# THUDM/GCC

Measured on NVIDIA H100. Metric: subgraphs/sec (MoCo pretrain step), higher is better.
Workload: dtype f32

## Files before the change

gcc_b200/csrc/gin_bwd.cu:

```cuda
#include "gin_common.cuh"
#include "tc_gemm.cuh"
#ifndef GCCB_EMU
#include <cuda_bf16.h>
#endif

namespace gccb {

template <int H>
__global__ void __launch_bounds__(256)
gin_pool_predict_bwd_kernel(GinDims d, const int32_t* __restrict__ node_off_v, int B,
                            const float* __restrict__ params, gccb_gin_layout_t lay,
                            const float* __restrict__ score, const float* __restrict__ dfeat,
                            uint64_t drop_key, uint64_t drop_step, int drop_layer_base,
                            uint32_t keep_thresh, int DW, float* __restrict__ dS,
                            float* __restrict__ dpool) {
  constexpr int G = GCCB_GPB;
  __shared__ float ds[G][H];
  __shared__ float dsl[G][H];
  const int g0 = blockIdx.x * G, tid = threadIdx.x, lane = tid & 31;
  const int ng = min(G, B - g0);
  if (node_off_v[B] < 0) return;
  for (int gi = tid >> 5; gi < G; gi += 8) {
    if (gi >= ng) {
      for (int o = lane; o < H; o += 32) ds[gi][o] = 0.f;
      continue;
    }
    const int g = g0 + gi;
    float ss = 0.f, dot = 0.f;
    for (int o = lane; o < H; o += 32) {
      const float x = score[(size_t)g * H + o];
      ss = fmaf(x, x, ss);
      dot = fmaf(x, dfeat[(size_t)g * H + o], dot);
    }
    ss = warp_sum(ss);
    dot = warp_sum(dot);
    const float nrm = sqrtf(ss);
    for (int o = lane; o < H; o += 32) {
      const float x = score[(size_t)g * H + o], gy = dfeat[(size_t)g * H + o];
      float dx;
      if (!d.norm) dx = gy;
      else if (nrm > d.norm_eps) dx = (gy - x * (dot / (nrm * nrm))) / nrm;
      else dx = gy / d.norm_eps;
      ds[gi][o] = dx;
    }
  }
  __syncthreads();
  for (int l = 0; l < d.L; ++l) {
    const int inf = l == 0 ? d.din : H;
    for (int i = tid; i < G * H; i += 256) {
      const int gi = i / H, o = i - gi * H;
      float v = ds[gi][o];
      if (gi < ng) {
        if (drop_layer_base >= 0) {
          const uint32_t e = (uint32_t)((g0 + gi) * H + o);
          u32x4 w = philox_at(drop_key, drop_step, e >> 2, 0, (uint32_t)(drop_layer_base + l), GCCB_TAG_DROPOUT);
          const uint32_t word = (e & 3u) == 0 ? w.x : (e & 3u) == 1 ? w.y : (e & 3u) == 2 ? w.z : w.w;
          v = word < keep_thresh ? v / (1.0f - d.drop_p) : 0.f;
        }
        dS[((size_t)l * B + g0 + gi) * H + o] = v;
      }
      dsl[gi][o] = v;
    }
    __syncthreads();
    const float* Wp = params + lay.wp[l];
    for (int k = tid; k < DW; k += 256) {
      float sg[G];
#pragma unroll
      for (int gi = 0; gi < G; ++gi) sg[gi] = 0.f;
      if (k < inf) {
#pragma unroll 4
        for (int o = 0; o < H; ++o) {
          const float w = Wp[(size_t)o * inf + k];
#pragma unroll
          for (int gi = 0; gi < G; ++gi) sg[gi] = fmaf(dsl[gi][o], w, sg[gi]);
        }
      }
#pragma unroll
      for (int gi = 0; gi < G; ++gi)
        if (gi < ng) dpool[((size_t)l * B + g0 + gi) * DW + k] = sg[gi];
    }
    __syncthreads();
  }
}

__global__ void __launch_bounds__(256)
gin_pred_wgrad_kernel(GinDims d, int B, gccb_gin_layout_t lay, const float* __restrict__ dS,
                      const float* __restrict__ pooled, int PW, float* __restrict__ grads) {
  const int l = blockIdx.y, H = d.H;
  const int inf = l == 0 ? d.din : H;
  const int idx = blockIdx.x * blockDim.x + threadIdx.x;
  if (idx < H * inf) {
    const int o = idx / inf, k = idx - o * inf;
    float s = 0.f;
    for (int g = 0; g < B; ++g)
      s = fmaf(dS[((size_t)l * B + g) * H + o], pooled[((size_t)l * B + g) * PW + k], s);
    grads[lay.wp[l] + idx] += s;
  } else if (idx < H * inf + H) {
    const int o = idx - H * inf;
    float s = 0.f;
    for (int g = 0; g < B; ++g) s += dS[((size_t)l * B + g) * H + o];
    grads[lay.bp[l] + o] += s;
  }
}

template <int W>
__global__ void __launch_bounds__(256)
gin_bwd_dh_kernel(const int32_t* __restrict__ node_off_v, int B, const int32_t* __restrict__ indptr,
                  const int32_t* __restrict__ indices, const int32_t* __restrict__ graph_id,
                  const float* __restrict__ dpool_j, int DW, const float* __restrict__ da, int has_da,
                  float* __restrict__ dh) {
  __shared__ float scratch[8 * W];
  __shared__ int hub_rows[GCCB_HUB_QUEUE];
  __shared__ int n_hub;
  const int N = node_off_v[B];
  const int tid = threadIdx.x, lane = tid & 31, warp = tid >> 5;
  constexpr int V4 = W / 4, PERV = (V4 + 31) / 32;
  if (tid == 0) n_hub = 0;
  __syncthreads();
  for (int r = blockIdx.x * 8 + warp; r < N; r += gridDim.x * 8) {
    const int beg = indptr[r], end = indptr[r + 1];
    if (has_da && end - beg > GCCB_HUB_DEG) {
      int slot = GCCB_HUB_QUEUE;
      if (lane == 0) slot = atomicAdd(&n_hub, 1);
      slot = __shfl_sync(0xffffffffu, slot, 0);
      if (slot < GCCB_HUB_QUEUE) {
        if (lane == 0) hub_rows[slot] = r;
        continue;
      }
    }
    const int g = graph_id[r];
    float4 acc[PERV];
#pragma unroll
    for (int j = 0; j < PERV; ++j) {
      const int v = lane + 32 * j;
      acc[j] = make_float4(0.f, 0.f, 0.f, 0.f);
      if (v < V4) {
        acc[j] = *reinterpret_cast<const float4*>(dpool_j + (size_t)g * DW + 4 * v);
        if (has_da) {
          const float4 x = *reinterpret_cast<const float4*>(da + (size_t)r * W + 4 * v);
          acc[j].x += x.x; acc[j].y += x.y; acc[j].z += x.z; acc[j].w += x.w;
        }
      }
    }
    if (has_da) gather_range4<W>(da, indices, beg, end, lane, acc);
#pragma unroll
    for (int j = 0; j < PERV; ++j) {
      const int v = lane + 32 * j;
      if (v < V4) *reinterpret_cast<float4*>(dh + (size_t)r * W + 4 * v) = acc[j];
    }
  }
  __syncthreads();
  const int nh = min(n_hub, GCCB_HUB_QUEUE);
  for (int hi = 0; hi < nh; ++hi) {
    const int rh = hub_rows[hi];
    const float s = gather_hub<W>(da, indices, indptr[rh], indptr[rh + 1], scratch);
    if (tid < W) dh[(size_t)rh * W + tid] = dpool_j[(size_t)graph_id[rh] * DW + tid] + da[(size_t)rh * W + tid] + s;
  }
}

struct BnC { const float *mean, *invstd, *sc, *sh; };
__device__ __forceinline__ BnC bnc(const float* p, int H) { BnC b; b.mean = p; b.invstd = p + H; b.sc = p + 2 * H; b.sh = p + 3 * H; return b; }

__device__ __forceinline__ void chain_g4(float z2v, float dhv, const BnC& A, const BnC& Bc, int c,
                                         float* ya, float* yhat, float* g4) {
  float yap = fmaf(z2v, A.sc[c], A.sh[c]);
  float y = fmaxf(yap, 0.f);
  float hb = fmaf(y, Bc.sc[c], Bc.sh[c]);
  *ya = yap;
  *yhat = (y - Bc.mean[c]) * Bc.invstd[c];
  *g4 = hb > 0.f ? dhv : 0.f;
}

template <int H>
__global__ void __launch_bounds__(256)
gin_bwd_reduce_kernel(int mode, const int32_t* __restrict__ node_off_v, int B,
                      const float* __restrict__ z2, const float* __restrict__ dh,
                      const double* __restrict__ sums_a, const float* __restrict__ ga,
                      const float* __restrict__ bea, const double* __restrict__ sums_b,
                      const float* __restrict__ gb, const float* __restrict__ beb, float bn_eps,
                      const double* __restrict__ redB_in, double* __restrict__ red_out) {
  __shared__ float coef_a[4 * H];
  __shared__ float coef_b[4 * H];
  __shared__ float red[2 * 1024];
  const int N = node_off_v[B];
  const int tid = threadIdx.x;
  bn_prepare(sums_a, N, H, ga, bea, bn_eps, coef_a, coef_a + H, coef_a + 2 * H, coef_a + 3 * H, nullptr, false, false, 0.f);
  bn_prepare(sums_b, N, H, gb, beb, bn_eps, coef_b, coef_b + H, coef_b + 2 * H, coef_b + 3 * H, nullptr, false, false, 0.f);
  __syncthreads();
  const BnC A = bnc(coef_a, H), Bc = bnc(coef_b, H);
  constexpr int TPR = H / 4, RP = 256 / TPR;
  const int c4 = (tid % TPR) * 4, rsub = tid / TPR;
  const float invN = N > 0 ? 1.0f / (float)N : 0.f;
  float m_g4[4] = {0.f, 0.f, 0.f, 0.f}, m_g4y[4] = {0.f, 0.f, 0.f, 0.f};
  if (mode == 1) {
#pragma unroll
    for (int k = 0; k < 4; ++k) { m_g4[k] = (float)(redB_in[c4 + k] * invN); m_g4y[k] = (float)(redB_in[H + c4 + k] * invN); }
  }
  float s[4] = {0.f, 0.f, 0.f, 0.f}, q[4] = {0.f, 0.f, 0.f, 0.f};
  const int stride = gridDim.x * RP;
  for (int r = blockIdx.x * RP + rsub; r < N; r += 2 * stride) {
    float4 zv[2], dv[2];
#pragma unroll
    for (int u = 0; u < 2; ++u) {
      const int rr = r + u * stride;
      const bool ok = rr < N;
      zv[u] = ok ? *reinterpret_cast<const float4*>(z2 + (size_t)rr * H + c4) : make_float4(0.f, 0.f, 0.f, 0.f);
      dv[u] = ok ? *reinterpret_cast<const float4*>(dh + (size_t)rr * H + c4) : make_float4(0.f, 0.f, 0.f, 0.f);
    }
#pragma unroll
    for (int u = 0; u < 2; ++u) {
      if (r + u * stride < N) {
        const float zz[4] = {zv[u].x, zv[u].y, zv[u].z, zv[u].w}, dd[4] = {dv[u].x, dv[u].y, dv[u].z, dv[u].w};
#pragma unroll
        for (int k = 0; k < 4; ++k) {
          const int c = c4 + k;
          float ya, yhat, g4;
          chain_g4(zz[k], dd[k], A, Bc, c, &ya, &yhat, &g4);
          if (mode == 0) {
            s[k] += g4;
            q[k] = fmaf(g4, yhat, q[k]);
          } else {
            const float dy = Bc.sc[c] * (g4 - m_g4[k] - yhat * m_g4y[k]);
            const float g3 = ya > 0.f ? dy : 0.f;
            const float z2hat = (zz[k] - A.mean[c]) * A.invstd[c];
            s[k] += g3;
            q[k] = fmaf(g3, z2hat, q[k]);
          }
        }
      }
    }
  }
#pragma unroll
  for (int k = 0; k < 4; ++k) {
    red[(0 * RP + rsub) * H + c4 + k] = s[k];
    red[(RP + rsub) * H + c4 + k] = q[k];
  }
  __syncthreads();
  for (int idx = tid; idx < 2 * H; idx += 256) {
    int which = idx / H, cc = idx - which * H;
    float t = 0.f;
    for (int j = 0; j < RP; ++j) t += red[(which * RP + j) * H + cc];
    atomicAdd(&red_out[which * H + cc], (double)t);
  }
}

template <int NOUT>
__device__ __forceinline__ void tile_colstats2(const float (&sv)[4][TileCols<NOUT>::CPT],
                                               const float (&qv)[4][TileCols<NOUT>::CPT], float* red,
                                               double* __restrict__ sums) {
  using TC = TileCols<NOUT>;
  const int tx = threadIdx.x & 15, ty = threadIdx.x >> 4;
#pragma unroll
  for (int c = 0; c < TC::CPT; ++c) {
    float s = 0.f, q = 0.f;
#pragma unroll
    for (int i = 0; i < 4; ++i) { s += sv[i][c]; q += qv[i][c]; }
    red[(0 * 16 + ty) * NOUT + TC::col(tx, c)] = s;
    red[(1 * 16 + ty) * NOUT + TC::col(tx, c)] = q;
  }
  __syncthreads();
  for (int idx = threadIdx.x; idx < 2 * NOUT; idx += blockDim.x) {
    int which = idx / NOUT, c = idx - which * NOUT;
    float s = 0.f;
#pragma unroll
    for (int t = 0; t < 16; ++t) s += red[(which * 16 + t) * NOUT + c];
    atomicAdd(&sums[which * NOUT + c], (double)s);
  }
  __syncthreads();
}

template <int H>
__global__ void __launch_bounds__(256)
gin_bwd_gemm2_kernel(const int32_t* __restrict__ node_off_v, int B, const float* __restrict__ z1,
                     const float* __restrict__ z2, const float* __restrict__ dh,
                     const double* __restrict__ sums_1, const float* __restrict__ g1w,
                     const float* __restrict__ be1, const double* __restrict__ sums_a,
                     const float* __restrict__ ga, const float* __restrict__ bea,
                     const double* __restrict__ sums_b, const float* __restrict__ gb,
                     const float* __restrict__ beb, float bn_eps, const double* __restrict__ redB,
                     const double* __restrict__ redA, const float* __restrict__ W2,
                     float* __restrict__ dz2_out, float* __restrict__ g1_out,
                     double* __restrict__ red1_out) {
  GCCB_DYN_SMEM(float, smem);
  constexpr int LDA = H + 1;
  float* As = smem;
  float* Ws = As + GCCB_TILE_ROWS * LDA;
  float* red = Ws + GCCB_KC * (H + 4);
  float* coef = red + 2 * 16 * H;
  float* rmean = coef + 12 * H;
  const int N = node_off_v[B];
  const int tid = threadIdx.x, tx = tid & 15, ty = tid >> 4;
  using TC = TileCols<H>;
  bn_prepare(sums_1, N, H, g1w, be1, bn_eps, coef, coef + H, coef + 2 * H, coef + 3 * H, nullptr, false, false, 0.f);
  bn_prepare(sums_a, N, H, ga, bea, bn_eps, coef + 4 * H, coef + 5 * H, coef + 6 * H, coef + 7 * H, nullptr, false, false, 0.f);
  bn_prepare(sums_b, N, H, gb, beb, bn_eps, coef + 8 * H, coef + 9 * H, coef + 10 * H, coef + 11 * H, nullptr, false, false, 0.f);
  const double invN = N > 0 ? 1.0 / (double)N : 0.0;
  for (int c = tid; c < H; c += 256) {
    rmean[c] = (float)(redB[c] * invN);
    rmean[H + c] = (float)(redB[H + c] * invN);
    rmean[2 * H + c] = (float)(redA[c] * invN);
    rmean[3 * H + c] = (float)(redA[H + c] * invN);
  }
  __syncthreads();
  const BnC C1 = bnc(coef, H), A = bnc(coef + 4 * H, H), Bc = bnc(coef + 8 * H, H);
  for (int tile = blockIdx.x; tile * GCCB_TILE_ROWS < N; tile += gridDim.x) {
    const int row0 = tile * GCCB_TILE_ROWS;
    __syncthreads();
#pragma unroll 8
    for (int idx = tid; idx < GCCB_TILE_ROWS * H; idx += 256) {
      int rr = idx / H, c = idx - rr * H;
      int r = row0 + rr;
      float dz = 0.f;
      if (r < N) {
        float ya, yhat, g4;
        float zv = z2[(size_t)r * H + c];
        chain_g4(zv, dh[(size_t)r * H + c], A, Bc, c, &ya, &yhat, &g4);
        float dy = Bc.sc[c] * (g4 - rmean[c] - yhat * rmean[H + c]);
        float g3 = ya > 0.f ? dy : 0.f;
        float z2hat = (zv - A.mean[c]) * A.invstd[c];
        dz = A.sc[c] * (g3 - rmean[2 * H + c] - z2hat * rmean[3 * H + c]);
        dz2_out[(size_t)r * H + c] = dz;
      }
      As[rr * LDA + c] = dz;
    }
    __syncthreads();
    float acc[4][TC::CPT];
    tile_gemm<H>(As, LDA, H, Ws, [&](int o, int k) { return W2[(size_t)o * H + k]; }, acc);
    float sv[4][TC::CPT], qv[4][TC::CPT];
#pragma unroll
    for (int i = 0; i < 4; ++i) {
      const int r = row0 + ty * 4 + i;
#pragma unroll
      for (int c = 0; c < TC::CPT; ++c) {
        const int col = TC::col(tx, c);
        float g = 0.f, gz = 0.f;
        if (r < N) {
          float zv = z1[(size_t)r * H + col];
          float pre = fmaf(zv, C1.sc[col], C1.sh[col]);
          g = pre > 0.f ? acc[i][c] : 0.f;
          gz = g * ((zv - C1.mean[col]) * C1.invstd[col]);
          g1_out[(size_t)r * H + col] = g;
        }
        sv[i][c] = g;
        qv[i][c] = gz;
      }
    }
    tile_colstats2<H>(sv, qv, red, red1_out);
  }
}

template <int KIN, int H>
__global__ void __launch_bounds__(256)
gin_bwd_gemm1_kernel(const int32_t* __restrict__ node_off_v, int B, const float* __restrict__ z1,
                     float* __restrict__ g1_dz1, const double* __restrict__ sums_1,
                     const float* __restrict__ g1w, const float* __restrict__ be1, float bn_eps,
                     const double* __restrict__ red1, const float* __restrict__ W1, int in_features,
                     float* __restrict__ da_out) {
  GCCB_DYN_SMEM(float, smem);
  constexpr int LDA = H + 1;
  float* As = smem;
  float* Ws = As + GCCB_TILE_ROWS * LDA;
  float* coef = Ws + GCCB_KC * (KIN + 4);
  float* rmean = coef + 4 * H;
  const int N = node_off_v[B];
  const int tid = threadIdx.x, tx = tid & 15, ty = tid >> 4;
  using TC = TileCols<KIN>;
  bn_prepare(sums_1, N, H, g1w, be1, bn_eps, coef, coef + H, coef + 2 * H, coef + 3 * H, nullptr, false, false, 0.f);
  const double invN = N > 0 ? 1.0 / (double)N : 0.0;
  for (int c = tid; c < H; c += 256) {
    rmean[c] = (float)(red1[c] * invN);
    rmean[H + c] = (float)(red1[H + c] * invN);
  }
  __syncthreads();
  const BnC C1 = bnc(coef, H);
  for (int tile = blockIdx.x; tile * GCCB_TILE_ROWS < N; tile += gridDim.x) {
    const int row0 = tile * GCCB_TILE_ROWS;
    __syncthreads();
#pragma unroll 8
    for (int idx = tid; idx < GCCB_TILE_ROWS * H; idx += 256) {
      int rr = idx / H, c = idx - rr * H;
      int r = row0 + rr;
      float dz = 0.f;
      if (r < N) {
        float zhat = (z1[(size_t)r * H + c] - C1.mean[c]) * C1.invstd[c];
        dz = C1.sc[c] * (g1_dz1[(size_t)r * H + c] - rmean[c] - zhat * rmean[H + c]);
        g1_dz1[(size_t)r * H + c] = dz;
      }
      As[rr * LDA + c] = dz;
    }
    __syncthreads();
    float acc[4][TC::CPT];
    tile_gemm<KIN>(As, LDA, H, Ws,
                   [&](int o, int k) { return k < in_features ? W1[(size_t)o * in_features + k] : 0.f; }, acc);
#pragma unroll
    for (int i = 0; i < 4; ++i) {
      const int r = row0 + ty * 4 + i;
      if (r < N) {
#pragma unroll
        for (int c = 0; c < TC::CPT; ++c) da_out[(size_t)r * KIN + TC::col(tx, c)] = acc[i][c];
      }
    }
  }
}

__global__ void __launch_bounds__(256)
gin_wgrad_kernel(const int32_t* __restrict__ node_off_v, int B, int H, int KQ,
                 const float* __restrict__ P, const float* __restrict__ Q,
                 const double* __restrict__ q_sums, const float* __restrict__ q_gamma,
                 const float* __restrict__ q_beta, float bn_eps, float* __restrict__ part) {
  __shared__ float Ps[GCCB_TILE_ROWS][65];
  __shared__ float Qs[GCCB_TILE_ROWS][65];
  __shared__ float qsc[64], qsh[64];
  const int N = node_off_v[B];
  const int tid = threadIdx.x, tx = tid & 15, ty = tid >> 4;
  const int kblocks = (KQ + 63) / 64;
  const int ob = blockIdx.y / kblocks, kb = blockIdx.y - ob * kblocks;
  const int o0 = ob * 64, k0 = kb * 64;
  const bool xform = q_sums != nullptr;
  if (xform) {
    for (int c = tid; c < 64; c += 256) {
      int k = k0 + c;
      float sc = 0.f, sh = 0.f;
      if (k < KQ) {
        double n = N > 0 ? (double)N : 1.0;
        double mean = q_sums[k] / n, var = q_sums[KQ + k] / n - mean * mean;
        if (var < 0.0) var = 0.0;
        float invstd = 1.0f / sqrtf((float)var + bn_eps);
        sc = q_gamma[k] * invstd;
        sh = q_beta[k] - (float)mean * sc;
      }
      qsc[c] = sc; qsh[c] = sh;
    }
  }
  __syncthreads();
  float acc[4][4];
  float bacc = 0.f;
#pragma unroll
  for (int i = 0; i < 4; ++i)
#pragma unroll
    for (int j = 0; j < 4; ++j) acc[i][j] = 0.f;
  const int tiles = (N + GCCB_TILE_ROWS - 1) / GCCB_TILE_ROWS;
  const int per = (tiles + GCCB_WG_CHUNKS - 1) / GCCB_WG_CHUNKS;
  const int t_beg = blockIdx.x * per, t_end = min(tiles, t_beg + per);
  for (int tile = t_beg; tile < t_end; ++tile) {
    const int row0 = tile * GCCB_TILE_ROWS;
    __syncthreads();
#pragma unroll 8
    for (int idx = tid; idx < GCCB_TILE_ROWS * 64; idx += 256) {
      int rr = idx >> 6, c = idx & 63;
      int r = row0 + rr;
      float pv = 0.f, qv = 0.f;
      if (r < N) {
        if (o0 + c < H) pv = P[(size_t)r * H + o0 + c];
        if (k0 + c < KQ) {
          qv = Q[(size_t)r * KQ + k0 + c];
          if (xform) qv = fmaxf(fmaf(qv, qsc[c], qsh[c]), 0.f);
        }
      }
      Ps[rr][c] = pv;
      Qs[rr][c] = qv;
    }
    __syncthreads();
    for (int rr = 0; rr < GCCB_TILE_ROWS; ++rr) {
      float p[4], q[4];
#pragma unroll
      for (int i = 0; i < 4; ++i) p[i] = Ps[rr][ty * 4 + i];
#pragma unroll
      for (int j = 0; j < 4; ++j) q[j] = Qs[rr][tx * 4 + j];
#pragma unroll
      for (int i = 0; i < 4; ++i)
#pragma unroll
        for (int j = 0; j < 4; ++j) acc[i][j] = fmaf(p[i], q[j], acc[i][j]);
    }
    if (kb == 0 && tid < 64)
      for (int rr = 0; rr < GCCB_TILE_ROWS; ++rr) bacc += Ps[rr][tid];
  }
  float* mypart = part + (size_t)blockIdx.x * ((size_t)H * KQ + H);
#pragma unroll
  for (int i = 0; i < 4; ++i) {
    int o = o0 + ty * 4 + i;
#pragma unroll
    for (int j = 0; j < 4; ++j) {
      int k = k0 + tx * 4 + j;
      if (o < H && k < KQ) mypart[(size_t)o * KQ + k] = acc[i][j];
    }
  }
  if (kb == 0 && tid < 64 && o0 + tid < H) mypart[(size_t)H * KQ + o0 + tid] = bacc;
}

__global__ void __launch_bounds__(256)
gin_wgrad_reduce_kernel(int H, int KQ, int in_features, const float* __restrict__ part,
                        float* __restrict__ gw, float* __restrict__ gb) {
  const int idx = blockIdx.x * blockDim.x + threadIdx.x;
  const size_t stride = (size_t)H * KQ + H;
  if (idx < H * KQ) {
    const int o = idx / KQ, k = idx - o * KQ;
    if (k < in_features) {
      float s0 = 0.f, s1 = 0.f, s2 = 0.f, s3 = 0.f;
      for (int ch = 0; ch < GCCB_WG_CHUNKS; ch += 4) {
        s0 += part[(ch + 0) * stride + idx]; s1 += part[(ch + 1) * stride + idx];
        s2 += part[(ch + 2) * stride + idx]; s3 += part[(ch + 3) * stride + idx];
      }
      gw[(size_t)o * in_features + k] += (s0 + s1) + (s2 + s3);
    }
  } else if (idx < H * KQ + H) {
    float s = 0.f;
    for (int ch = 0; ch < GCCB_WG_CHUNKS; ++ch) s += part[ch * stride + idx];
    gb[idx - H * KQ] += s;
  }
}

__global__ void gin_bn_grads_kernel(int H, const double* __restrict__ red, float* __restrict__ gw,
                                    float* __restrict__ gb) {
  int c = blockIdx.x * blockDim.x + threadIdx.x;
  if (c < H) { gb[c] += (float)red[c]; gw[c] += (float)red[H + c]; }
}

__global__ void __launch_bounds__(256)
gin_bwd_emb_kernel(GinDims d, const int32_t* __restrict__ node_off_v, int B,
                   const int32_t* __restrict__ sub_deg, const float* __restrict__ dx0,
                   float* __restrict__ gemb) {
  GCCB_DYN_SMEM(float, hist);
  const int N = node_off_v[B];
  const int cells = (d.maxdeg + 1) * d.D;
  for (int i = threadIdx.x; i < cells; i += blockDim.x) hist[i] = 0.f;
  __syncthreads();
  const int total = N * d.D;
  for (int idx = blockIdx.x * blockDim.x + threadIdx.x; idx < total; idx += gridDim.x * blockDim.x) {
    int r = idx / d.D, c = idx - r * d.D;
    int dg = sub_deg[r];
    dg = dg < 0 ? 0 : (dg > d.maxdeg ? d.maxdeg : dg);
    atomicAdd(&hist[dg * d.D + c], dx0[(size_t)r * GCCB_DINP + d.P + c]);
  }
  __syncthreads();
  for (int i = threadIdx.x; i < cells; i += blockDim.x) {
    float v = hist[i];
    if (v != 0.f) atomicAdd(&gemb[i], v);
  }
}

struct BwdArgs {
  GinDims d;
  const gccb_batch_t* batch;
  int view;
  const float* params;
  gccb_gin_layout_t lay;
  const char* acts;
  ActsLayout al;
  const float* dfeat;
  float* grads;
  char* ws;
  BwdLayout bl;
  uint64_t drop_key, drop_step;
  int drop_base;
  gccb_stream_t stream;
};

template <int H>
static int run_backward(const BwdArgs& a) {
  const GinDims& d = a.d;
  const int B = a.batch->batch, cap = a.batch->node_cap;
  const int32_t* node_off_v = a.batch->node_off + (size_t)a.view * (B + 1);
  const int32_t* indptr = a.batch->indptr + (size_t)a.view * (cap + 1);
  const int32_t* indices = a.batch->indices + (size_t)a.view * a.batch->edge_cap;
  const int32_t* sub_deg = a.batch->sub_deg + (size_t)a.view * cap;
  const int32_t* graph_id = a.batch->graph_id + (size_t)a.view * cap;
  const double* stats = (const double*)(a.acts + a.al.stats);
  float* dh = (float*)(a.ws + a.bl.dh);
  float* da = (float*)(a.ws + a.bl.da);
  double* red = (double*)(a.ws + a.bl.red);
  float* dS = (float*)(a.ws + a.bl.dS);
  float* dpool = (float*)(a.ws + a.bl.dpool);
  float* part = (float*)(a.ws + a.bl.part);
  const float* P = a.params;
  float* G = a.grads;
  const int DW = a.bl.DW;
  const int tiles = (cap + GCCB_TILE_ROWS - 1) / GCCB_TILE_ROWS;
  const int grid = tiles < 4 * GCCB_NUM_SMS ? tiles : 4 * GCCB_NUM_SMS;
  const uint32_t keep = (uint32_t)fmin((1.0 - (double)d.drop_p) * 4294967296.0, 4294967295.0);
#ifndef GCCB_EMU
  StreamKit* kit = stream_kit((cudaStream_t)a.stream, 1);
  cudaStream_t main_s = (cudaStream_t)a.stream;
  gccb_stream_t side = kit->side[0];
  cudaEvent_t* ev_main = kit->ev;
  cudaEvent_t* ev_side = kit->ev + 8;
  cudaEvent_t ev_head = kit->ev[16], ev_join = kit->ev[17];
#else
  gccb_stream_t side = a.stream;
#endif
  cudaMemsetAsync(red, 0, (size_t)(d.L - 1) * 3 * 2 * H * sizeof(double), (cudaStream_t)a.stream);
  auto kpb = gin_pool_predict_bwd_kernel<H>;
  GCCB_LAUNCH(kpb, (B + GCCB_GPB - 1) / GCCB_GPB, 256, 0, a.stream, d, node_off_v, B, P, a.lay, (const float*)(a.acts + a.al.score),
              a.dfeat, a.drop_key, a.drop_step, a.drop_base, keep, DW, dS, dpool);
#ifndef GCCB_EMU
  cudaEventRecord(ev_head, main_s);
  cudaStreamWaitEvent((cudaStream_t)side, ev_head, 0);
#endif
  {
    int maxout = H * (d.din > H ? d.din : H) + H;
    dim3 gr((maxout + 255) / 256, d.L);
    GCCB_LAUNCH(gin_pred_wgrad_kernel, gr, 256, 0, side, d, B, a.lay, (const float*)dS,
                (const float*)(a.acts + a.al.pooled), a.al.PW, G);
  }
  for (int l = d.L - 2; l >= 0; --l) {
    float* g1 = (float*)(a.ws + a.bl.g1[l & 1]);
    float* dz2 = (float*)(a.ws + a.bl.dz2[l & 1]);
    const int j = l + 1;
    const float* z1 = (const float*)(a.acts + a.al.z1[l]);
    const float* z2 = (const float*)(a.acts + a.al.z2[l]);
    const float* a_l = (const float*)(a.acts + a.al.a[l]);
    const double* s1 = stats + (size_t)(l * 3 + 0) * 2 * H;
    const double* sa = stats + (size_t)(l * 3 + 1) * 2 * H;
    const double* sb = stats + (size_t)(l * 3 + 2) * 2 * H;
    double* r1 = red + (size_t)(l * 3 + 0) * 2 * H;
    double* rA = red + (size_t)(l * 3 + 1) * 2 * H;
    double* rB = red + (size_t)(l * 3 + 2) * 2 * H;
    auto kdh = gin_bwd_dh_kernel<H>;
    GCCB_LAUNCH(kdh, (tiles < 1184 ? tiles : 1184), 256, 0, a.stream, node_off_v, B, indptr, indices, graph_id,
                (const float*)(dpool + (size_t)j * B * DW), DW, (const float*)da, j < d.L - 1 ? 1 : 0, dh);
    auto kred = gin_bwd_reduce_kernel<H>;
    GCCB_LAUNCH(kred, grid, 256, 0, a.stream, 0, node_off_v, B, z2, (const float*)dh, sa, P + a.lay.bna_w[l],
                P + a.lay.bna_b[l], sb, P + a.lay.bnb_w[l], P + a.lay.bnb_b[l], d.bn_eps,
                (const double*)rB, rB);
    GCCB_LAUNCH(kred, grid, 256, 0, a.stream, 1, node_off_v, B, z2, (const float*)dh, sa, P + a.lay.bna_w[l],
                P + a.lay.bna_b[l], sb, P + a.lay.bnb_w[l], P + a.lay.bnb_b[l], d.bn_eps,
                (const double*)rB, rA);
#ifndef GCCB_EMU
    if (l + 2 <= d.L - 2) cudaStreamWaitEvent(main_s, ev_side[l + 2], 0);
#endif
    {
      auto k = gin_bwd_gemm2_kernel<H>;
      size_t sm = ((size_t)GCCB_TILE_ROWS * (H + 1) + (size_t)GCCB_KC * (H + 4) + 2 * 16 * H + 16 * H) * 4;
      gccb::ensure_dyn_smem(k, sm);
      GCCB_LAUNCH(k, grid, 256, sm, a.stream, node_off_v, B, z1, z2, (const float*)dh, s1, P + a.lay.bn1_w[l],
                  P + a.lay.bn1_b[l], sa, P + a.lay.bna_w[l], P + a.lay.bna_b[l], sb, P + a.lay.bnb_w[l],
                  P + a.lay.bnb_b[l], d.bn_eps, (const double*)rB, (const double*)rA, P + a.lay.w2[l], dz2,
                  g1, r1);
    }
    const int KQ1 = gin_in_width(d, l), inf = gin_in_features(d, l);
    if (l == 0) {
      auto k = gin_bwd_gemm1_kernel<GCCB_DINP, H>;
      size_t sm = ((size_t)GCCB_TILE_ROWS * (H + 1) + (size_t)GCCB_KC * (GCCB_DINP + 4) + 6 * H) * 4;
      gccb::ensure_dyn_smem(k, sm);
      GCCB_LAUNCH(k, grid, 256, sm, a.stream, node_off_v, B, z1, g1, s1, P + a.lay.bn1_w[l], P + a.lay.bn1_b[l],
                  d.bn_eps, (const double*)r1, P + a.lay.w1[l], inf, da);
    } else {
      auto k = gin_bwd_gemm1_kernel<H, H>;
      size_t sm = ((size_t)GCCB_TILE_ROWS * (H + 1) + (size_t)GCCB_KC * (H + 4) + 6 * H) * 4;
      gccb::ensure_dyn_smem(k, sm);
      GCCB_LAUNCH(k, grid, 256, sm, a.stream, node_off_v, B, z1, g1, s1, P + a.lay.bn1_w[l], P + a.lay.bn1_b[l],
                  d.bn_eps, (const double*)r1, P + a.lay.w1[l], inf, da);
    }
#ifndef GCCB_EMU
    cudaEventRecord(ev_main[l], main_s);
    cudaStreamWaitEvent((cudaStream_t)side, ev_main[l], 0);
#endif
    {
      dim3 gr(GCCB_WG_CHUNKS, ((H + 63) / 64) * ((H + 63) / 64));
      GCCB_LAUNCH(gin_wgrad_kernel, gr, 256, 0, side, node_off_v, B, H, H, (const float*)dz2, z1, s1,
                  P + a.lay.bn1_w[l], P + a.lay.bn1_b[l], d.bn_eps, part);
      GCCB_LAUNCH(gin_wgrad_reduce_kernel, (H * H + H + 255) / 256, 256, 0, side, H, H, H,
                  (const float*)part, G + a.lay.w2[l], G + a.lay.b2[l]);
      dim3 gr1(GCCB_WG_CHUNKS, ((H + 63) / 64) * ((KQ1 + 63) / 64));
      GCCB_LAUNCH(gin_wgrad_kernel, gr1, 256, 0, side, node_off_v, B, H, KQ1, (const float*)g1, a_l,
                  (const double*)nullptr, (const float*)nullptr, (const float*)nullptr, d.bn_eps, part);
      GCCB_LAUNCH(gin_wgrad_reduce_kernel, (H * KQ1 + H + 255) / 256, 256, 0, side, H, KQ1, inf,
                  (const float*)part, G + a.lay.w1[l], G + a.lay.b1[l]);
    }
    GCCB_LAUNCH(gin_bn_grads_kernel, (H + 127) / 128, 128, 0, side, H, (const double*)rB,
                G + a.lay.bnb_w[l], G + a.lay.bnb_b[l]);
    GCCB_LAUNCH(gin_bn_grads_kernel, (H + 127) / 128, 128, 0, side, H, (const double*)rA,
                G + a.lay.bna_w[l], G + a.lay.bna_b[l]);
    GCCB_LAUNCH(gin_bn_grads_kernel, (H + 127) / 128, 128, 0, side, H, (const double*)r1,
                G + a.lay.bn1_w[l], G + a.lay.bn1_b[l]);
#ifndef GCCB_EMU
    cudaEventRecord(ev_side[l], (cudaStream_t)side);
#endif
  }
  auto kdh0 = gin_bwd_dh_kernel<GCCB_DINP>;
  GCCB_LAUNCH(kdh0, (tiles < 1184 ? tiles : 1184), 256, 0, a.stream, node_off_v, B, indptr, indices, graph_id, (const float*)dpool, DW,
              (const float*)da, 1, dh);
  {
    size_t sm = (size_t)(d.maxdeg + 1) * d.D * sizeof(float);
    auto k = gin_bwd_emb_kernel;
    gccb::ensure_dyn_smem(k, sm);
    GCCB_LAUNCH(k, 64, 256, sm, a.stream, d, node_off_v, B, sub_deg, (const float*)dh, G + a.lay.emb);
  }
#ifndef GCCB_EMU
  cudaEventRecord(ev_join, (cudaStream_t)side);
  cudaStreamWaitEvent(main_s, ev_join, 0);
#endif
  return check_launch("gccb_gin_backward");
}


#ifndef GCCB_EMU

template <int H>
__global__ void __launch_bounds__(256)
gin_bwd_dz2_kernel(const int32_t* __restrict__ node_off_v, int B, const float* __restrict__ z2,
                   const float* __restrict__ dh, const double* __restrict__ sums_1, const float* __restrict__ g1w,
                   const float* __restrict__ be1, const double* __restrict__ sums_a, const float* __restrict__ ga,
                   const float* __restrict__ bea, const double* __restrict__ sums_b, const float* __restrict__ gb,
                   const float* __restrict__ beb, float bn_eps, const double* __restrict__ redB,
                   const double* __restrict__ redA, float* __restrict__ dz2_out, __nv_bfloat16* __restrict__ dz16,
                   float* __restrict__ coef1_out) {
  __shared__ float coef[12 * H];
  __shared__ float rmean[4 * H];
  const int N = node_off_v[B];
  const int tid = threadIdx.x;
  bn_prepare(sums_1, N, H, g1w, be1, bn_eps, coef, coef + H, coef + 2 * H, coef + 3 * H, nullptr, false, false, 0.f);
  bn_prepare(sums_a, N, H, ga, bea, bn_eps, coef + 4 * H, coef + 5 * H, coef + 6 * H, coef + 7 * H, nullptr, false, false, 0.f);
  bn_prepare(sums_b, N, H, gb, beb, bn_eps, coef + 8 * H, coef + 9 * H, coef + 10 * H, coef + 11 * H, nullptr, false, false, 0.f);
  const double invN = N > 0 ? 1.0 / (double)N : 0.0;
  for (int c = tid; c < H; c += 256) {
    rmean[c] = (float)(redB[c] * invN);
    rmean[H + c] = (float)(redB[H + c] * invN);
    rmean[2 * H + c] = (float)(redA[c] * invN);
    rmean[3 * H + c] = (float)(redA[H + c] * invN);
  }
  __syncthreads();
  if (blockIdx.x == 0)
    for (int c = tid; c < H; c += 256) { coef1_out[c] = coef[2 * H + c]; coef1_out[H + c] = coef[3 * H + c]; }
  const BnC A = bnc(coef + 4 * H, H), Bc = bnc(coef + 8 * H, H);
  const size_t total4 = (size_t)(N > 0 ? N : 0) * (H / 4);
  const size_t gstride = (size_t)gridDim.x * blockDim.x;
  for (size_t i0 = (size_t)blockIdx.x * blockDim.x + tid; i0 < total4; i0 += 2 * gstride) {
    float4 zv[2], dv[2];
#pragma unroll
    for (int u = 0; u < 2; ++u) {
      const size_t i = i0 + u * gstride;
      const bool ok = i < total4;
      zv[u] = ok ? reinterpret_cast<const float4*>(z2)[i] : make_float4(0.f, 0.f, 0.f, 0.f);
      dv[u] = ok ? reinterpret_cast<const float4*>(dh)[i] : make_float4(0.f, 0.f, 0.f, 0.f);
    }
#pragma unroll
    for (int u = 0; u < 2; ++u) {
      const size_t i = i0 + u * gstride;
      if (i < total4) {
        const int c0 = (int)(i % (H / 4)) * 4;
        const float zz[4] = {zv[u].x, zv[u].y, zv[u].z, zv[u].w}, dd[4] = {dv[u].x, dv[u].y, dv[u].z, dv[u].w};
        float o[4];
#pragma unroll
        for (int k = 0; k < 4; ++k) {
          const int c = c0 + k;
          float ya, yhat, g4;
          chain_g4(zz[k], dd[k], A, Bc, c, &ya, &yhat, &g4);
          const float dy = Bc.sc[c] * (g4 - rmean[c] - yhat * rmean[H + c]);
          const float g3 = ya > 0.f ? dy : 0.f;
          const float z2hat = (zz[k] - A.mean[c]) * A.invstd[c];
          o[k] = A.sc[c] * (g3 - rmean[2 * H + c] - z2hat * rmean[3 * H + c]);
        }
        reinterpret_cast<float4*>(dz2_out)[i] = make_float4(o[0], o[1], o[2], o[3]);
        const __nv_bfloat162 p0 = __floats2bfloat162_rn(o[0], o[1]), p1 = __floats2bfloat162_rn(o[2], o[3]);
        uint2 w;
        w.x = *reinterpret_cast<const uint32_t*>(&p0);
        w.y = *reinterpret_cast<const uint32_t*>(&p1);
        reinterpret_cast<uint2*>(dz16)[i] = w;
      }
    }
  }
}

template <int H>
__global__ void __launch_bounds__(256)
gin_bwd_g1_kernel(const int32_t* __restrict__ node_off_v, int B, const float* __restrict__ z1,
                  float* __restrict__ dx1_g1, const double* __restrict__ sums_1, const float* __restrict__ g1w,
                  const float* __restrict__ be1, float bn_eps, double* __restrict__ red1_out) {
  __shared__ float coef[4 * H];
  __shared__ float red[2 * 1024];
  const int N = node_off_v[B];
  const int tid = threadIdx.x;
  bn_prepare(sums_1, N, H, g1w, be1, bn_eps, coef, coef + H, coef + 2 * H, coef + 3 * H, nullptr, false, false, 0.f);
  __syncthreads();
  const BnC C1 = bnc(coef, H);
  constexpr int TPR = H / 4, RP = 256 / TPR;
  const int c4 = (tid % TPR) * 4, rsub = tid / TPR;
  float s[4] = {0.f, 0.f, 0.f, 0.f}, q[4] = {0.f, 0.f, 0.f, 0.f};
  const int stride = gridDim.x * RP;
  for (int r = blockIdx.x * RP + rsub; r < N; r += 2 * stride) {
    float4 zv[2], dv[2];
#pragma unroll
    for (int u = 0; u < 2; ++u) {
      const int rr = r + u * stride;
      const bool ok = rr < N;
      zv[u] = ok ? *reinterpret_cast<const float4*>(z1 + (size_t)rr * H + c4) : make_float4(0.f, 0.f, 0.f, 0.f);
      dv[u] = ok ? *reinterpret_cast<const float4*>(dx1_g1 + (size_t)rr * H + c4) : make_float4(0.f, 0.f, 0.f, 0.f);
    }
#pragma unroll
    for (int u = 0; u < 2; ++u) {
      const int rr = r + u * stride;
      if (rr < N) {
        const float zz[4] = {zv[u].x, zv[u].y, zv[u].z, zv[u].w}, dd[4] = {dv[u].x, dv[u].y, dv[u].z, dv[u].w};
        float o[4];
#pragma unroll
        for (int k = 0; k < 4; ++k) {
          const int c = c4 + k;
          const float pre = fmaf(zz[k], C1.sc[c], C1.sh[c]);
          o[k] = pre > 0.f ? dd[k] : 0.f;
          s[k] += o[k];
          q[k] = fmaf(o[k], (zz[k] - C1.mean[c]) * C1.invstd[c], q[k]);
        }
        *reinterpret_cast<float4*>(dx1_g1 + (size_t)rr * H + c4) = make_float4(o[0], o[1], o[2], o[3]);
      }
    }
  }
#pragma unroll
  for (int k = 0; k < 4; ++k) {
    red[(0 * RP + rsub) * H + c4 + k] = s[k];
    red[(RP + rsub) * H + c4 + k] = q[k];
  }
  __syncthreads();
  for (int idx = tid; idx < 2 * H; idx += 256) {
    const int which = idx / H, cc = idx - which * H;
    float t = 0.f;
    for (int j = 0; j < RP; ++j) t += red[(which * RP + j) * H + cc];
    atomicAdd(&red1_out[which * H + cc], (double)t);
  }
}

template <int H>
__global__ void __launch_bounds__(256)
gin_bwd_dz1_kernel(const int32_t* __restrict__ node_off_v, int B, const float* __restrict__ z1,
                   float* __restrict__ g1_dz1, const double* __restrict__ sums_1, const float* __restrict__ g1w,
                   const float* __restrict__ be1, float bn_eps, const double* __restrict__ red1,
                   __nv_bfloat16* __restrict__ dz16) {
  __shared__ float coef[4 * H];
  __shared__ float rmean[2 * H];
  const int N = node_off_v[B];
  const int tid = threadIdx.x;
  bn_prepare(sums_1, N, H, g1w, be1, bn_eps, coef, coef + H, coef + 2 * H, coef + 3 * H, nullptr, false, false, 0.f);
  const double invN = N > 0 ? 1.0 / (double)N : 0.0;
  for (int c = tid; c < H; c += 256) {
    rmean[c] = (float)(red1[c] * invN);
    rmean[H + c] = (float)(red1[H + c] * invN);
  }
  __syncthreads();
  const BnC C1 = bnc(coef, H);
  const size_t total4 = (size_t)(N > 0 ? N : 0) * (H / 4);
  const size_t gstride = (size_t)gridDim.x * blockDim.x;
  for (size_t i0 = (size_t)blockIdx.x * blockDim.x + tid; i0 < total4; i0 += 2 * gstride) {
    float4 zv[2], gv[2];
#pragma unroll
    for (int u = 0; u < 2; ++u) {
      const size_t i = i0 + u * gstride;
      const bool ok = i < total4;
      zv[u] = ok ? reinterpret_cast<const float4*>(z1)[i] : make_float4(0.f, 0.f, 0.f, 0.f);
      gv[u] = ok ? reinterpret_cast<const float4*>(g1_dz1)[i] : make_float4(0.f, 0.f, 0.f, 0.f);
    }
#pragma unroll
    for (int u = 0; u < 2; ++u) {
      const size_t i = i0 + u * gstride;
      if (i < total4) {
        const int c0 = (int)(i % (H / 4)) * 4;
        const float zz[4] = {zv[u].x, zv[u].y, zv[u].z, zv[u].w}, gg[4] = {gv[u].x, gv[u].y, gv[u].z, gv[u].w};
        float o[4];
#pragma unroll
        for (int k = 0; k < 4; ++k) {
          const int c = c0 + k;
          const float zhat = (zz[k] - C1.mean[c]) * C1.invstd[c];
          o[k] = C1.sc[c] * (gg[k] - rmean[c] - zhat * rmean[H + c]);
        }
        reinterpret_cast<float4*>(g1_dz1)[i] = make_float4(o[0], o[1], o[2], o[3]);
        const __nv_bfloat162 p0 = __floats2bfloat162_rn(o[0], o[1]), p1 = __floats2bfloat162_rn(o[2], o[3]);
        uint2 w;
        w.x = *reinterpret_cast<const uint32_t*>(&p0);
        w.y = *reinterpret_cast<const uint32_t*>(&p1);
        reinterpret_cast<uint2*>(dz16)[i] = w;
      }
    }
  }
}

template <int H>
static int run_backward_tc(const BwdArgs& a) {
  const GinDims& d = a.d;
  const int B = a.batch->batch, cap = a.batch->node_cap;
  const int32_t* node_off_v = a.batch->node_off + (size_t)a.view * (B + 1);
  const int32_t* n_dev = node_off_v + B;
  const int32_t* indptr = a.batch->indptr + (size_t)a.view * (cap + 1);
  const int32_t* indices = a.batch->indices + (size_t)a.view * a.batch->edge_cap;
  const int32_t* sub_deg = a.batch->sub_deg + (size_t)a.view * cap;
  const int32_t* graph_id = a.batch->graph_id + (size_t)a.view * cap;
  const double* stats = (const double*)(a.acts + a.al.stats);
  float* dh = (float*)(a.ws + a.bl.dh);
  float* da = (float*)(a.ws + a.bl.da);
  double* red = (double*)(a.ws + a.bl.red);
  float* dS = (float*)(a.ws + a.bl.dS);
  float* dpool = (float*)(a.ws + a.bl.dpool);
  __nv_bfloat16* dz16 = (__nv_bfloat16*)(a.ws + a.bl.dz16);
  __nv_bfloat16* tA = (__nv_bfloat16*)(a.ws + a.bl.tA);
  __nv_bfloat16* tB = (__nv_bfloat16*)(a.ws + a.bl.tB);
  float* coef1 = (float*)(a.ws + a.bl.coef1);
  float* splitk = (float*)(a.ws + a.bl.splitk);
  const float* P = a.params;
  float* G = a.grads;
  const int DW = a.bl.DW, capP = a.bl.cap_pad;
  const int tiles = (cap + GCCB_TILE_ROWS - 1) / GCCB_TILE_ROWS;
  const int grid = tiles < 4 * GCCB_NUM_SMS ? tiles : 4 * GCCB_NUM_SMS;
  const uint32_t keep = (uint32_t)fmin((1.0 - (double)d.drop_p) * 4294967296.0, 4294967295.0);
  StreamKit* kit = stream_kit((cudaStream_t)a.stream, 1);
  cudaStream_t main_s = (cudaStream_t)a.stream;
  cudaStream_t side = kit->side[0];
  cudaEvent_t* ev_main = kit->ev;
  cudaEvent_t* ev_side = kit->ev + 8;
  cudaEvent_t ev_head = kit->ev[16], ev_join = kit->ev[17];
  cudaMemsetAsync(red, 0, (size_t)(d.L - 1) * 3 * 2 * H * sizeof(double), main_s);
  auto kpb = gin_pool_predict_bwd_kernel<H>;
  GCCB_LAUNCH(kpb, (B + GCCB_GPB - 1) / GCCB_GPB, 256, 0, a.stream, d, node_off_v, B, P, a.lay, (const float*)(a.acts + a.al.score),
              a.dfeat, a.drop_key, a.drop_step, a.drop_base, keep, DW, dS, dpool);
  cudaEventRecord(ev_head, main_s);
  cudaStreamWaitEvent(side, ev_head, 0);
  {
    int maxout = H * (d.din > H ? d.din : H) + H;
    dim3 gr((maxout + 255) / 256, d.L);
    GCCB_LAUNCH(gin_pred_wgrad_kernel, gr, 256, 0, side, d, B, a.lay, (const float*)dS,
                (const float*)(a.acts + a.al.pooled), a.al.PW, G);
  }
  for (int l = d.L - 2; l >= 0; --l) {
    float* g1 = (float*)(a.ws + a.bl.g1[l & 1]);
    float* dz2 = (float*)(a.ws + a.bl.dz2[l & 1]);
    const int j = l + 1;
    const float* z1 = (const float*)(a.acts + a.al.z1[l]);
    const float* z2 = (const float*)(a.acts + a.al.z2[l]);
    const float* a_l = (const float*)(a.acts + a.al.a[l]);
    const double* s1 = stats + (size_t)(l * 3 + 0) * 2 * H;
    const double* sa = stats + (size_t)(l * 3 + 1) * 2 * H;
    const double* sb = stats + (size_t)(l * 3 + 2) * 2 * H;
    double* r1 = red + (size_t)(l * 3 + 0) * 2 * H;
    double* rA = red + (size_t)(l * 3 + 1) * 2 * H;
    double* rB = red + (size_t)(l * 3 + 2) * 2 * H;
    const int KW = gin_kw(d, l), inf = gin_in_features(d, l);
    const __nv_bfloat16* w1b = (const __nv_bfloat16*)(a.acts + a.al.w16[l]);
    const __nv_bfloat16* w1t = w1b + (size_t)H * KW + (size_t)H * H;
    const __nv_bfloat16* w2t = w1t + (size_t)KW * H;
    float* c1 = coef1 + (size_t)l * 2 * H;
    auto kdh = gin_bwd_dh_kernel<H>;
    GCCB_LAUNCH(kdh, (tiles < 1184 ? tiles : 1184), 256, 0, a.stream, node_off_v, B, indptr, indices, graph_id,
                (const float*)(dpool + (size_t)j * B * DW), DW, (const float*)da, j < d.L - 1 ? 1 : 0, dh);
    auto kred = gin_bwd_reduce_kernel<H>;
    GCCB_LAUNCH(kred, grid, 256, 0, a.stream, 0, node_off_v, B, z2, (const float*)dh, sa, P + a.lay.bna_w[l],
                P + a.lay.bna_b[l], sb, P + a.lay.bnb_w[l], P + a.lay.bnb_b[l], d.bn_eps, (const double*)rB, rB);
    GCCB_LAUNCH(kred, grid, 256, 0, a.stream, 1, node_off_v, B, z2, (const float*)dh, sa, P + a.lay.bna_w[l],
                P + a.lay.bna_b[l], sb, P + a.lay.bnb_w[l], P + a.lay.bnb_b[l], d.bn_eps, (const double*)rB, rA);
    if (l + 2 <= d.L - 2) cudaStreamWaitEvent(main_s, ev_side[l + 2], 0);
    auto kz2 = gin_bwd_dz2_kernel<H>;
    GCCB_LAUNCH(kz2, grid, 256, 0, a.stream, node_off_v, B, z2, (const float*)dh, s1, P + a.lay.bn1_w[l],
                P + a.lay.bn1_b[l], sa, P + a.lay.bna_w[l], P + a.lay.bna_b[l], sb, P + a.lay.bnb_w[l],
                P + a.lay.bnb_b[l], d.bn_eps, (const double*)rB, (const double*)rA, dz2, dz16, c1);
    int rc = tc::gemm_bf16(dz16, w2t, cap, H, H, n_dev, nullptr, 1.0f, g1, nullptr, H, nullptr, 1, nullptr, main_s);
    if (rc) return rc;
    auto kg1 = gin_bwd_g1_kernel<H>;
    GCCB_LAUNCH(kg1, grid, 256, 0, a.stream, node_off_v, B, z1, g1, s1, P + a.lay.bn1_w[l], P + a.lay.bn1_b[l],
                d.bn_eps, r1);
    auto kz1 = gin_bwd_dz1_kernel<H>;
    GCCB_LAUNCH(kz1, grid, 256, 0, a.stream, node_off_v, B, z1, g1, s1, P + a.lay.bn1_w[l], P + a.lay.bn1_b[l],
                d.bn_eps, (const double*)r1, dz16);
    rc = tc::gemm_bf16(dz16, w1t, cap, KW, H, n_dev, nullptr, 1.0f, da, nullptr, KW, nullptr, 1, nullptr, main_s);
    if (rc) return rc;
    cudaEventRecord(ev_main[l], main_s);
    cudaStreamWaitEvent(side, ev_main[l], 0);
    rc = tc::cast_bf16(dz2, cap, H, H, tA, capP, H, 1, n_dev, side);
    if (!rc) rc = tc::cast_bf16(z1, cap, H, H, tB, capP, H, 1, n_dev, side, c1, c1 + H, 1);
    if (!rc) rc = tc::gemm_bf16(tA, tB, H, H, capP, nullptr, nullptr, 1.0f, G + a.lay.w2[l], nullptr, H, nullptr,
                                a.bl.splits, splitk, side, 1.0f, H);
    if (!rc) rc = tc::cast_bf16(g1, cap, H, H, tA, capP, H, 1, n_dev, side);
    if (!rc) rc = tc::cast_bf16(a_l, cap, KW, KW, tB, capP, KW, 1, n_dev, side);
    if (!rc) rc = tc::gemm_bf16(tA, tB, H, KW, capP, nullptr, nullptr, 1.0f, G + a.lay.w1[l], nullptr, inf, nullptr,
                                a.bl.splits, splitk, side, 1.0f, inf);
    if (rc) return rc;
    GCCB_LAUNCH(gin_bn_grads_kernel, (H + 127) / 128, 128, 0, side, H, (const double*)rB,
                G + a.lay.bnb_w[l], G + a.lay.bnb_b[l]);
    GCCB_LAUNCH(gin_bn_grads_kernel, (H + 127) / 128, 128, 0, side, H, (const double*)rA,
                G + a.lay.bna_w[l], G + a.lay.bna_b[l]);
    GCCB_LAUNCH(gin_bn_grads_kernel, (H + 127) / 128, 128, 0, side, H, (const double*)r1,
                G + a.lay.bn1_w[l], G + a.lay.bn1_b[l]);
    cudaEventRecord(ev_side[l], side);
  }
  auto kdh0 = gin_bwd_dh_kernel<GCCB_DINP>;
  GCCB_LAUNCH(kdh0, (tiles < 1184 ? tiles : 1184), 256, 0, a.stream, node_off_v, B, indptr, indices, graph_id, (const float*)dpool, DW,
              (const float*)da, 1, dh);
  {
    size_t sm = (size_t)(d.maxdeg + 1) * d.D * sizeof(float);
    auto k = gin_bwd_emb_kernel;
    gccb::ensure_dyn_smem(k, sm);
    GCCB_LAUNCH(k, 64, 256, sm, a.stream, d, node_off_v, B, sub_deg, (const float*)dh, G + a.lay.emb);
  }
  cudaEventRecord(ev_join, side);
  cudaStreamWaitEvent(main_s, ev_join, 0);
  return check_launch("gccb_gin_backward (tensor cores)");
}
#endif

}

using namespace gccb;

extern "C" size_t gccb_gin_backward_workspace(const gccb_gin_cfg_t* cfg, int32_t batch, int32_t node_cap) {
  GinDims d;
  if (dims_from_cfg(cfg, &d)) return 0;
  return make_bwd_layout(d, batch, node_cap).total;
}

extern "C" int gccb_gin_stash_layout(const gccb_gin_cfg_t* cfg, int32_t batch, int32_t node_cap,
                                     gccb_gin_stash_t* out) {
  GinDims d;
  int rc = dims_from_cfg(cfg, &d);
  if (rc) return rc;
  if (!out || batch < 1 || node_cap < 1) {
    set_last_error("gccb_gin_stash_layout: bad argument");
    return GCCB_ERR_BADARG;
  }
  const ActsLayout al = make_acts_layout(d, batch, node_cap);
  const BwdLayout bl = make_bwd_layout(d, batch, node_cap);
  auto tc = [&](size_t off) { return d.tc ? (int64_t)off : (int64_t)-1; };
  out->x0 = (int64_t)al.x0;
  for (int l = 0; l < 8; ++l) {
    const bool live = l < d.L - 1;
    out->a[l] = live ? (int64_t)al.a[l] : -1;
    out->z1[l] = live ? (int64_t)al.z1[l] : -1;
    out->z2[l] = live ? (int64_t)al.z2[l] : -1;
    out->h[l] = live ? (int64_t)al.h[l] : -1;
    out->w16[l] = live ? tc(al.w16[l]) : -1;
  }
  out->stats = (int64_t)al.stats;
  out->pooled = (int64_t)al.pooled;
  out->a16 = tc(al.a16);
  out->x16 = tc(al.x16);
  out->dh = (int64_t)bl.dh;
  for (int i = 0; i < 2; ++i) {
    out->g1[i] = (int64_t)bl.g1[i];
    out->dz2[i] = (int64_t)bl.dz2[i];
  }
  out->da = (int64_t)bl.da;
  out->dpool = (int64_t)bl.dpool;
  out->coef1 = tc(bl.coef1);
  out->dz16 = tc(bl.dz16);
  out->tA = tc(bl.tA);
  out->tB = tc(bl.tB);
  out->cap_pad = d.tc ? bl.cap_pad : -1;
  out->splits = d.tc ? bl.splits : -1;
  out->DW = bl.DW;
  out->PW = al.PW;
  return GCCB_OK;
}

extern "C" int gccb_gin_backward(const gccb_gin_cfg_t* cfg, const gccb_batch_t* batch, int32_t view,
                                 const float* params, const void* acts, const float* dfeat, float* grads,
                                 uint64_t dropout_key, uint64_t dropout_step,
                                 int32_t dropout_layer_base, void* workspace, size_t workspace_bytes,
                                 gccb_stream_t stream) {
  BwdArgs a;
  int rc = dims_from_cfg(cfg, &a.d);
  if (rc) return rc;
  if (!batch || !params || !acts || !dfeat || !grads || !workspace || view < 0 || view > 1) {
    set_last_error("gccb_gin_backward: bad argument");
    return GCCB_ERR_BADARG;
  }
  a.al = make_acts_layout(a.d, batch->batch, batch->node_cap);
  a.bl = make_bwd_layout(a.d, batch->batch, batch->node_cap);
  if (workspace_bytes < a.bl.total) {
    set_last_error("gccb_gin_backward: workspace too small");
    return GCCB_ERR_CAPACITY;
  }
  make_param_layout(a.d, &a.lay);
  a.batch = batch; a.view = view; a.params = params; a.acts = (const char*)acts; a.dfeat = dfeat;
  a.grads = grads; a.ws = (char*)workspace; a.stream = stream;
  a.drop_key = dropout_key; a.drop_step = dropout_step; a.drop_base = dropout_layer_base;
#ifndef GCCB_EMU
  if (a.d.tc) return a.d.H == 128 ? run_backward_tc<128>(a) : run_backward_tc<256>(a);
#endif
  switch (a.d.H) {
    case 32: return run_backward<32>(a);
    case 64: return run_backward<64>(a);
    case 128: return run_backward<128>(a);
    default: return run_backward<256>(a);
  }
}
```

gcc_b200/csrc/gin_common.cuh:

```cuda
#pragma once
#include "common.cuh"

namespace gccb {

#define GCCB_DINP 64
#define GCCB_TILE_ROWS 64
#define GCCB_KC 64
#define GCCB_MAX_L 8

struct GinDims {
  int L, H, P, D, maxdeg, din;
  int norm;
  int tc;
  float bn_eps, bn_mom, norm_eps, drop_p;
};

__host__ __device__ __forceinline__ int gin_in_features(const GinDims& d, int l) { return l == 0 ? d.din : d.H; }
__host__ __device__ __forceinline__ int gin_in_width(const GinDims& d, int l) { return l == 0 ? GCCB_DINP : d.H; }

struct ActsLayout {
  size_t x0;
  size_t a[GCCB_MAX_L], z1[GCCB_MAX_L], z2[GCCB_MAX_L], h[GCCB_MAX_L];
  size_t stats;
  size_t pool_acc;
  size_t pooled;
  size_t score;
  size_t feat;
  size_t a16;
  size_t x16;
  size_t w16[GCCB_MAX_L];
  size_t total;
  int PW;
};
__host__ __device__ __forceinline__ int gin_kw(const GinDims& d, int l) { return l == 0 ? GCCB_DINP : d.H; }
inline size_t gin_w16_elems(const GinDims& d, int l) { return (size_t)2 * d.H * gin_kw(d, l) + (size_t)2 * d.H * d.H; }

inline ActsLayout make_acts_layout(const GinDims& d, int B, int node_cap) {
  ActsLayout a;
  size_t off = 0;
  auto take = [&](size_t bytes) { size_t o = off; off += (bytes + 255) & ~(size_t)255; return o; };
  a.x0 = take((size_t)node_cap * GCCB_DINP * 4);
  for (int l = 0; l < GCCB_MAX_L; ++l) a.a[l] = a.z1[l] = a.z2[l] = a.h[l] = 0;
  for (int l = 0; l < d.L - 1; ++l) {
    a.a[l] = take((size_t)node_cap * gin_in_width(d, l) * 4);
    a.z1[l] = take((size_t)node_cap * d.H * 4);
    a.z2[l] = take((size_t)node_cap * d.H * 4);
    a.h[l] = take((size_t)node_cap * d.H * 4);
  }
  a.stats = take((size_t)(d.L - 1) * 3 * 2 * d.H * 8);
  a.PW = d.H > GCCB_DINP ? d.H : GCCB_DINP;
  a.pool_acc = take((size_t)d.L * B * a.PW * 8);
  a.pooled = take((size_t)d.L * B * a.PW * 4);
  a.score = take((size_t)B * d.H * 4);
  a.feat = take((size_t)B * d.H * 4);
  a.a16 = a.x16 = 0;
  for (int l = 0; l < GCCB_MAX_L; ++l) a.w16[l] = 0;
  if (d.tc) {
    a.a16 = take((size_t)node_cap * (d.H > GCCB_DINP ? d.H : GCCB_DINP) * 2);
    a.x16 = take((size_t)node_cap * d.H * 2);
    for (int l = 0; l < d.L - 1; ++l) a.w16[l] = take(gin_w16_elems(d, l) * 2);
  }
  a.total = off;
  return a;
}

#define GCCB_WG_CHUNKS GCCB_NUM_SMS

struct BwdLayout {
  size_t dh, g1[2], dz2[2], da, red, dS, dpool, part, total;
  size_t dz16, tA, tB, coef1, splitk;
  int DW;
  int cap_pad, splits;
};

inline BwdLayout make_bwd_layout(const GinDims& d, int B, int node_cap) {
  BwdLayout b;
  size_t off = 0;
  auto take = [&](size_t bytes) { size_t o = off; off += (bytes + 255) & ~(size_t)255; return o; };
  b.DW = d.H > GCCB_DINP ? d.H : GCCB_DINP;
  b.dh = take((size_t)node_cap * b.DW * 4);
  for (int i = 0; i < 2; ++i) {
    b.g1[i] = take((size_t)node_cap * d.H * 4);
    b.dz2[i] = take((size_t)node_cap * d.H * 4);
  }
  b.da = take((size_t)node_cap * b.DW * 4);
  b.red = take((size_t)(d.L - 1) * 3 * 2 * d.H * 8);
  b.dS = take((size_t)d.L * B * d.H * 4);
  b.dpool = take((size_t)d.L * B * b.DW * 4);
  b.part = take((size_t)GCCB_WG_CHUNKS * ((size_t)d.H * b.DW + d.H) * 4);
  b.dz16 = b.tA = b.tB = b.coef1 = b.splitk = 0;
  b.cap_pad = (node_cap + 63) & ~63;
  b.splits = 0;
#ifndef GCCB_EMU
  if (d.tc) {
    b.dz16 = take((size_t)node_cap * d.H * 2);
    b.tA = take((size_t)d.H * b.cap_pad * 2);
    b.tB = take((size_t)b.DW * b.cap_pad * 2);
    b.coef1 = take((size_t)(d.L - 1) * 2 * d.H * 4);
    const int tiles = (d.H / 128) * 1;
    b.splits = GCCB_NUM_SMS / tiles;
    if (b.splits > b.cap_pad / 64) b.splits = b.cap_pad / 64;
    if (b.splits < 1) b.splits = 1;
    b.splitk = take((size_t)b.splits * d.H * b.DW * 4);
  }
#endif
  b.total = off;
  return b;
}

inline void make_param_layout(const GinDims& d, gccb_gin_layout_t* o) {
  int64_t off = 0;
  auto take = [&](int64_t n) { int64_t r = off; off += n; return r; };
  for (int l = 0; l < 8; ++l)
    o->w1[l] = o->b1[l] = o->bn1_w[l] = o->bn1_b[l] = o->w2[l] = o->b2[l] = o->bna_w[l] = o->bna_b[l] =
        o->bnb_w[l] = o->bnb_b[l] = o->wp[l] = o->bp[l] = -1;
  for (int l = 0; l < d.L - 1; ++l) {
    o->w1[l] = take((int64_t)d.H * gin_in_features(d, l));
    o->b1[l] = take(d.H);
    o->bn1_w[l] = take(d.H);
    o->bn1_b[l] = take(d.H);
    o->w2[l] = take((int64_t)d.H * d.H);
    o->b2[l] = take(d.H);
    o->bna_w[l] = take(d.H);
    o->bna_b[l] = take(d.H);
    o->bnb_w[l] = take(d.H);
    o->bnb_b[l] = take(d.H);
  }
  for (int l = 0; l < d.L; ++l) {
    o->wp[l] = take((int64_t)d.H * gin_in_features(d, l));
    o->bp[l] = take(d.H);
  }
  o->emb = take((int64_t)(d.maxdeg + 1) * d.D);
  o->total = off;
  o->run_total = (int64_t)(d.L - 1) * 3 * 2 * d.H;
}

inline int dims_from_cfg(const gccb_gin_cfg_t* c, GinDims* d) {
  if (!c) return GCCB_ERR_BADARG;
  d->L = c->num_layers; d->H = c->hidden; d->P = c->pos_dim; d->D = c->deg_dim;
  d->maxdeg = c->max_degree; d->din = c->pos_dim + c->deg_dim + 1; d->norm = c->norm;
  d->bn_eps = c->bn_eps; d->bn_mom = c->bn_momentum; d->norm_eps = c->norm_eps; d->drop_p = c->dropout_p;
#ifdef GCCB_EMU
  d->tc = 0;
#else
  d->tc = (c->tensor_cores && c->hidden >= 128) ? 1 : 0;
#endif
  if (d->L < 2 || d->L > GCCB_MAX_L || (d->H != 32 && d->H != 64 && d->H != 128 && d->H != 256) ||
      d->din > GCCB_DINP || d->P < 2 || d->P > 32 || d->D < 1 || d->maxdeg < 1) {
    set_last_error("gin: unsupported configuration (L=%d H=%d pos=%d deg=%d): need 2<=L<=8, "
                   "H in {32,64,128,256}, pos+deg+1<=64, pos<=32", d->L, d->H, d->P, d->D);
    return GCCB_ERR_BADARG;
  }
  return GCCB_OK;
}

__device__ __forceinline__ void bn_prepare(const double* __restrict__ sums, int N, int H,
                                           const float* __restrict__ gamma,
                                           const float* __restrict__ beta, float eps,
                                           float* mean_s, float* invstd_s, float* sc_s, float* sh_s,
                                           float* __restrict__ running ,
                                           bool use_running, bool update_running, float momentum) {
  for (int c = threadIdx.x; c < H; c += blockDim.x) {
    double mean, var;
    if (use_running) {
      mean = running[c];
      var = running[H + c];
    } else {
      double n = N > 0 ? (double)N : 1.0;
      mean = sums[c] / n;
      var = sums[H + c] / n - mean * mean;
      if (var < 0.0) var = 0.0;
      if (update_running && running && blockIdx.x == 0 && N > 0) {
        double unb = N > 1 ? var * n / (n - 1.0) : var;
        running[c] = (float)((1.0 - momentum) * running[c] + momentum * mean);
        running[H + c] = (float)((1.0 - momentum) * running[H + c] + momentum * unb);
      }
    }
    float invstd = 1.0f / sqrtf((float)var + eps);
    float g = gamma[c];
    mean_s[c] = (float)mean;
    invstd_s[c] = invstd;
    sc_s[c] = g * invstd;
    sh_s[c] = beta[c] - (float)mean * g * invstd;
  }
}

#ifndef GCCB_HUB_DEG
#define GCCB_HUB_DEG 256
#endif
#define GCCB_GPB 8
#define GCCB_HUB_QUEUE 64
template <int W>
__device__ __forceinline__ void gather_range(const float* __restrict__ src, const int32_t* __restrict__ indices,
                                             int beg, int end, int lane, float (&acc)[(W + 31) / 32]) {
  constexpr int PER = (W + 31) / 32;
  int e = beg;
  for (; e + 7 < end; e += 8) {
    int u[8];
#pragma unroll
    for (int k = 0; k < 8; ++k) u[k] = indices[e + k];
#pragma unroll
    for (int j = 0; j < PER; ++j) {
      const int c = lane + 32 * j;
      if (c < W) {
        float x[8];
#pragma unroll
        for (int k = 0; k < 8; ++k) x[k] = src[(size_t)u[k] * W + c];
        acc[j] += ((x[0] + x[1]) + (x[2] + x[3])) + ((x[4] + x[5]) + (x[6] + x[7]));
      }
    }
  }
  for (; e < end; ++e) {
    const int u = indices[e];
#pragma unroll
    for (int j = 0; j < PER; ++j) {
      const int c = lane + 32 * j;
      if (c < W) acc[j] += src[(size_t)u * W + c];
    }
  }
}

template <int W>
__device__ __forceinline__ void gather_range4(const float* __restrict__ src, const int32_t* __restrict__ indices,
                                              int beg, int end, int lane, float4 (&acc)[(W / 4 + 31) / 32]) {
  constexpr int V4 = W / 4, PERV = (V4 + 31) / 32;
  int e = beg;
  for (; e + 3 < end; e += 4) {
    const int u0 = indices[e], u1 = indices[e + 1], u2 = indices[e + 2], u3 = indices[e + 3];
#pragma unroll
    for (int j = 0; j < PERV; ++j) {
      const int v = lane + 32 * j;
      if (v < V4) {
        const float4 x0 = *reinterpret_cast<const float4*>(src + (size_t)u0 * W + 4 * v);
        const float4 x1 = *reinterpret_cast<const float4*>(src + (size_t)u1 * W + 4 * v);
        const float4 x2 = *reinterpret_cast<const float4*>(src + (size_t)u2 * W + 4 * v);
        const float4 x3 = *reinterpret_cast<const float4*>(src + (size_t)u3 * W + 4 * v);
        acc[j].x += (x0.x + x1.x) + (x2.x + x3.x);
        acc[j].y += (x0.y + x1.y) + (x2.y + x3.y);
        acc[j].z += (x0.z + x1.z) + (x2.z + x3.z);
        acc[j].w += (x0.w + x1.w) + (x2.w + x3.w);
      }
    }
  }
  for (; e < end; ++e) {
    const int u = indices[e];
#pragma unroll
    for (int j = 0; j < PERV; ++j) {
      const int v = lane + 32 * j;
      if (v < V4) {
        const float4 x = *reinterpret_cast<const float4*>(src + (size_t)u * W + 4 * v);
        acc[j].x += x.x; acc[j].y += x.y; acc[j].z += x.z; acc[j].w += x.w;
      }
    }
  }
}

template <int W>
__device__ __forceinline__ float gather_hub(const float* __restrict__ src, const int32_t* __restrict__ indices,
                                            int beg, int end, float* scratch) {
  constexpr int PER = (W + 31) / 32;
  const int lane = threadIdx.x & 31, warp = threadIdx.x >> 5;
  const int len = end - beg, per = (len + 7) / 8;
  const int b = beg + warp * per, e = min(b + per, end);
  float acc[PER];
#pragma unroll
  for (int j = 0; j < PER; ++j) acc[j] = 0.f;
  gather_range<W>(src, indices, b, e > b ? e : b, lane, acc);
#pragma unroll
  for (int j = 0; j < PER; ++j) {
    const int c = lane + 32 * j;
    if (c < W) scratch[warp * W + c] = acc[j];
  }
  __syncthreads();
  float s = 0.f;
  if ((int)threadIdx.x < W) {
#pragma unroll
    for (int w = 0; w < 8; ++w) s += scratch[w * W + threadIdx.x];
  }
  __syncthreads();
  return s;
}

template <int NOUT> struct TileCols {
  static constexpr int CPT = NOUT / 16;
  static constexpr int VEC = CPT < 4 ? CPT : 4;
  __device__ static __forceinline__ int col(int tx, int c) { return (c / VEC) * (16 * VEC) + tx * VEC + (c % VEC); }
};

template <int NOUT, class GetW>
__device__ __forceinline__ void stage_weights(float* Ws, int k0, int kc, GetW getw) {
  constexpr int LDW = NOUT + 4;
#pragma unroll 8
  for (int idx = threadIdx.x; idx < kc * NOUT; idx += blockDim.x) {
    int kk = idx % kc, c = idx / kc;
    Ws[kk * LDW + c] = getw(k0 + kk, c);
  }
}

template <int NOUT>
__device__ __forceinline__ void tile_mma(const float* As, int lda, int k0, int kc, const float* Ws,
                                         float (&acc)[4][TileCols<NOUT>::CPT]) {
  using TC = TileCols<NOUT>;
  constexpr int LDW = NOUT + 4;
  const int tx = threadIdx.x & 15, ty = threadIdx.x >> 4;
  for (int kk = 0; kk < kc; ++kk) {
    float a[4];
#pragma unroll
    for (int i = 0; i < 4; ++i) a[i] = As[(ty * 4 + i) * lda + k0 + kk];
    float w[TC::CPT];
#pragma unroll
    for (int c = 0; c < TC::CPT; ++c) w[c] = Ws[kk * LDW + TC::col(tx, c)];
#pragma unroll
    for (int i = 0; i < 4; ++i)
#pragma unroll
      for (int c = 0; c < TC::CPT; ++c) acc[i][c] = fmaf(a[i], w[c], acc[i][c]);
  }
}

template <int NOUT, class GetW>
__device__ __forceinline__ void tile_gemm(const float* As, int lda, int K, float* Ws, GetW getw,
                                          float (&acc)[4][TileCols<NOUT>::CPT]) {
#pragma unroll
  for (int i = 0; i < 4; ++i)
#pragma unroll
    for (int c = 0; c < TileCols<NOUT>::CPT; ++c) acc[i][c] = 0.f;
  for (int k0 = 0; k0 < K; k0 += GCCB_KC) {
    int kc = K - k0 < GCCB_KC ? K - k0 : GCCB_KC;
    __syncthreads();
    stage_weights<NOUT>(Ws, k0, kc, getw);
    __syncthreads();
    tile_mma<NOUT>(As, lda, k0, kc, Ws, acc);
  }
}

template <int NOUT>
__device__ __forceinline__ void tile_colstats(const float (&v)[4][TileCols<NOUT>::CPT], float* red ,
                                              double* __restrict__ sums) {
  using TC = TileCols<NOUT>;
  const int tx = threadIdx.x & 15, ty = threadIdx.x >> 4;
#pragma unroll
  for (int c = 0; c < TC::CPT; ++c) {
    float s = 0.f, q = 0.f;
#pragma unroll
    for (int i = 0; i < 4; ++i) { s += v[i][c]; q = fmaf(v[i][c], v[i][c], q); }
    red[(0 * 16 + ty) * NOUT + TC::col(tx, c)] = s;
    red[(1 * 16 + ty) * NOUT + TC::col(tx, c)] = q;
  }
  __syncthreads();
  for (int idx = threadIdx.x; idx < 2 * NOUT; idx += blockDim.x) {
    int which = idx / NOUT, c = idx - which * NOUT;
    float s = 0.f;
#pragma unroll
    for (int t = 0; t < 16; ++t) s += red[(which * 16 + t) * NOUT + c];
    atomicAdd(&sums[which * NOUT + c], (double)s);
  }
  __syncthreads();
}

}
```

gcc_b200/csrc/gin_fwd.cu:

```cuda
#include "gin_common.cuh"
#include "tc_gemm.cuh"
#ifndef GCCB_EMU
#include <cuda_bf16.h>
#endif

namespace gccb {

__global__ void __launch_bounds__(256)
gin_build_x0_kernel(GinDims d, const int32_t* __restrict__ node_off_v, int B,
                    const float* __restrict__ pos, const int32_t* __restrict__ sub_deg,
                    const int32_t* __restrict__ graph_id, const float* __restrict__ emb,
                    float* __restrict__ x0) {
  const int N = node_off_v[B];
  const int total = N * GCCB_DINP;
  for (int idx = blockIdx.x * blockDim.x + threadIdx.x; idx < total; idx += gridDim.x * blockDim.x) {
    int r = idx / GCCB_DINP, c = idx - r * GCCB_DINP;
    float v = 0.f;
    if (c < d.P) {
      v = pos[(size_t)r * d.P + c];
    } else if (c < d.P + d.D) {
      int dg = sub_deg[r];
      dg = dg < 0 ? 0 : (dg > d.maxdeg ? d.maxdeg : dg);
      v = emb[(size_t)dg * d.D + (c - d.P)];
    } else if (c == d.P + d.D) {
      v = (r == node_off_v[graph_id[r]]) ? 1.0f : 0.f;
    }
    x0[idx] = v;
  }
}

template <int KIN, int H>
__global__ void __launch_bounds__(256)
gin_agg_gemm1_kernel(const int32_t* __restrict__ node_off_v, int B, const int32_t* __restrict__ indptr,
                     const int32_t* __restrict__ indices, const float* __restrict__ h,
                     const float* __restrict__ W1, int in_features, const float* __restrict__ b1,
                     float eps_gin, float* __restrict__ a_out, float* __restrict__ z1,
                     double* __restrict__ sums) {
  GCCB_DYN_SMEM(float, smem);
  constexpr int LDA = KIN + 1;
  float* As = smem;
  float* Ws = As + GCCB_TILE_ROWS * LDA;
  float* red = Ws + GCCB_KC * (H + 4);
  __shared__ int hub_rows[GCCB_TILE_ROWS];
  __shared__ int n_hub;
  static_assert(8 * KIN <= 2 * 16 * H, "hub scratch must fit in the statistics scratch");
  const int N = node_off_v[B];
  const int tid = threadIdx.x, lane = tid & 31, warp = tid >> 5;
  const int tx = tid & 15, ty = tid >> 4;
  using TC = TileCols<H>;
  for (int tile = blockIdx.x; tile * GCCB_TILE_ROWS < N; tile += gridDim.x) {
    const int row0 = tile * GCCB_TILE_ROWS;
    __syncthreads();
    if (tid == 0) n_hub = 0;
    __syncthreads();
    for (int rr = warp; rr < GCCB_TILE_ROWS; rr += 8) {
      const int r = row0 + rr;
      constexpr int PER = (KIN + 31) / 32;
      float acc[PER];
#pragma unroll
      for (int j = 0; j < PER; ++j) acc[j] = 0.f;
      if (r < N) {
        const int beg = indptr[r], end = indptr[r + 1];
        if (end - beg > GCCB_HUB_DEG) {
          if (lane == 0) hub_rows[atomicAdd(&n_hub, 1)] = rr;
          continue;
        }
#pragma unroll
        for (int j = 0; j < PER; ++j) {
          int c = lane + 32 * j;
          if (c < KIN) acc[j] = (1.0f + eps_gin) * h[(size_t)r * KIN + c];
        }
        gather_range<KIN>(h, indices, beg, end, lane, acc);
      }
#pragma unroll
      for (int j = 0; j < PER; ++j) {
        int c = lane + 32 * j;
        if (c < KIN) {
          As[rr * LDA + c] = acc[j];
          if (r < N) a_out[(size_t)r * KIN + c] = acc[j];
        }
      }
    }
    __syncthreads();
    for (int hi = 0; hi < n_hub; ++hi) {
      const int rr = hub_rows[hi], r = row0 + rr;
      const float s = gather_hub<KIN>(h, indices, indptr[r], indptr[r + 1], red);
      if (tid < KIN) {
        const float v = (1.0f + eps_gin) * h[(size_t)r * KIN + tid] + s;
        As[rr * LDA + tid] = v;
        a_out[(size_t)r * KIN + tid] = v;
      }
    }
    __syncthreads();
    float acc[4][TC::CPT];
    tile_gemm<H>(As, LDA, KIN, Ws,
                 [&](int k, int o) { return k < in_features ? W1[(size_t)o * in_features + k] : 0.f; }, acc);
    float v[4][TC::CPT];
#pragma unroll
    for (int i = 0; i < 4; ++i) {
      const int r = row0 + ty * 4 + i;
#pragma unroll
      for (int c = 0; c < TC::CPT; ++c) {
        const int col = TC::col(tx, c);
        float z = acc[i][c] + b1[col];
        v[i][c] = r < N ? z : 0.f;
        if (r < N) z1[(size_t)r * H + col] = z;
      }
    }
    tile_colstats<H>(v, red, sums);
  }
}

template <int H>
__global__ void __launch_bounds__(256)
gin_bn_gemm2_kernel(const int32_t* __restrict__ node_off_v, int B, const float* __restrict__ z1,
                    const double* __restrict__ sums1, const float* __restrict__ g1,
                    const float* __restrict__ be1, float bn_eps, float* __restrict__ running1,
                    int use_running, int update_running, float momentum,
                    const float* __restrict__ W2, const float* __restrict__ b2,
                    float* __restrict__ z2, double* __restrict__ sums2) {
  GCCB_DYN_SMEM(float, smem);
  constexpr int LDA = H + 1;
  float* As = smem;
  float* Ws = As + GCCB_TILE_ROWS * LDA;
  float* red = Ws + GCCB_KC * (H + 4);
  float* coef = red + 2 * 16 * H;
  const int N = node_off_v[B];
  const int tid = threadIdx.x, tx = tid & 15, ty = tid >> 4;
  using TC = TileCols<H>;
  bn_prepare(sums1, N, H, g1, be1, bn_eps, coef, coef + H, coef + 2 * H, coef + 3 * H, running1,
             use_running != 0, update_running != 0, momentum);
  __syncthreads();
  const float* sc = coef + 2 * H;
  const float* sh = coef + 3 * H;
  for (int tile = blockIdx.x; tile * GCCB_TILE_ROWS < N; tile += gridDim.x) {
    const int row0 = tile * GCCB_TILE_ROWS;
    __syncthreads();
#pragma unroll 8
    for (int idx = tid; idx < GCCB_TILE_ROWS * H; idx += 256) {
      int rr = idx / H, c = idx - rr * H;
      int r = row0 + rr;
      float x = 0.f;
      if (r < N) x = fmaxf(fmaf(z1[(size_t)r * H + c], sc[c], sh[c]), 0.f);
      As[rr * LDA + c] = x;
    }
    __syncthreads();
    float acc[4][TC::CPT];
    tile_gemm<H>(As, LDA, H, Ws, [&](int k, int o) { return W2[(size_t)o * H + k]; }, acc);
    float v[4][TC::CPT];
#pragma unroll
    for (int i = 0; i < 4; ++i) {
      const int r = row0 + ty * 4 + i;
#pragma unroll
      for (int c = 0; c < TC::CPT; ++c) {
        const int col = TC::col(tx, c);
        float z = acc[i][c] + b2[col];
        v[i][c] = r < N ? z : 0.f;
        if (r < N) z2[(size_t)r * H + col] = z;
      }
    }
    tile_colstats<H>(v, red, sums2);
  }
}

template <int H>
__global__ void __launch_bounds__(256)
gin_bn_tail_kernel(int mode, const int32_t* __restrict__ node_off_v, int B,
                   const float* __restrict__ z2, const double* __restrict__ sums_a,
                   const float* __restrict__ ga, const float* __restrict__ bea,
                   float* __restrict__ running_a, const double* __restrict__ sums_b_in,
                   const float* __restrict__ gb, const float* __restrict__ beb,
                   float* __restrict__ running_b, float bn_eps, int use_running, int update_running,
                   float momentum, double* __restrict__ sums_b_out, float* __restrict__ h_out) {
  __shared__ float coef_a[4 * H];
  __shared__ float coef_b[4 * H];
  __shared__ float red[2 * 1024];
  const int N = node_off_v[B];
  const int tid = threadIdx.x;
  bn_prepare(sums_a, N, H, ga, bea, bn_eps, coef_a, coef_a + H, coef_a + 2 * H, coef_a + 3 * H,
             running_a, use_running != 0, update_running != 0 && mode == 0, momentum);
  if (mode == 1)
    bn_prepare(sums_b_in, N, H, gb, beb, bn_eps, coef_b, coef_b + H, coef_b + 2 * H, coef_b + 3 * H,
               running_b, use_running != 0, update_running != 0, momentum);
  __syncthreads();
  constexpr int TPR = H / 4, RP = 256 / TPR;
  const int c4 = (tid % TPR) * 4, rsub = tid / TPR;
  float sca[4], sha[4];
#pragma unroll
  for (int k = 0; k < 4; ++k) { sca[k] = coef_a[2 * H + c4 + k]; sha[k] = coef_a[3 * H + c4 + k]; }
  const int stride = gridDim.x * RP;
  if (mode == 0) {
    float s[4] = {0.f, 0.f, 0.f, 0.f}, q[4] = {0.f, 0.f, 0.f, 0.f};
    for (int r = blockIdx.x * RP + rsub; r < N; r += 4 * stride) {
      float4 z[4];
#pragma unroll
      for (int u = 0; u < 4; ++u) {
        const int rr = r + u * stride;
        z[u] = rr < N ? *reinterpret_cast<const float4*>(z2 + (size_t)rr * H + c4) : make_float4(0.f, 0.f, 0.f, 0.f);
      }
#pragma unroll
      for (int u = 0; u < 4; ++u) {
        if (r + u * stride < N) {
          const float zz[4] = {z[u].x, z[u].y, z[u].z, z[u].w};
#pragma unroll
          for (int k = 0; k < 4; ++k) {
            const float y = fmaxf(fmaf(zz[k], sca[k], sha[k]), 0.f);
            s[k] += y;
            q[k] = fmaf(y, y, q[k]);
          }
        }
      }
    }
#pragma unroll
    for (int k = 0; k < 4; ++k) {
      red[(0 * RP + rsub) * H + c4 + k] = s[k];
      red[(RP + rsub) * H + c4 + k] = q[k];
    }
    __syncthreads();
    for (int idx = tid; idx < 2 * H; idx += 256) {
      int which = idx / H, cc = idx - which * H;
      float t = 0.f;
      for (int j = 0; j < RP; ++j) t += red[(which * RP + j) * H + cc];
      atomicAdd(&sums_b_out[which * H + cc], (double)t);
    }
  } else {
    float scb[4], shb[4];
#pragma unroll
    for (int k = 0; k < 4; ++k) { scb[k] = coef_b[2 * H + c4 + k]; shb[k] = coef_b[3 * H + c4 + k]; }
    for (int r = blockIdx.x * RP + rsub; r < N; r += 4 * stride) {
      float4 z[4];
#pragma unroll
      for (int u = 0; u < 4; ++u) {
        const int rr = r + u * stride;
        z[u] = rr < N ? *reinterpret_cast<const float4*>(z2 + (size_t)rr * H + c4) : make_float4(0.f, 0.f, 0.f, 0.f);
      }
#pragma unroll
      for (int u = 0; u < 4; ++u) {
        const int rr = r + u * stride;
        if (rr < N) {
          const float zz[4] = {z[u].x, z[u].y, z[u].z, z[u].w};
          float o[4];
#pragma unroll
          for (int k = 0; k < 4; ++k) {
            const float y = fmaxf(fmaf(zz[k], sca[k], sha[k]), 0.f);
            o[k] = fmaxf(fmaf(y, scb[k], shb[k]), 0.f);
          }
          *reinterpret_cast<float4*>(h_out + (size_t)rr * H + c4) = make_float4(o[0], o[1], o[2], o[3]);
        }
      }
    }
  }
}

template <int H>
__global__ void __launch_bounds__(256)
gin_pool_kernel(int L, const int32_t* __restrict__ node_off_v, int B, const int32_t* __restrict__ graph_id,
                const float* __restrict__ x0, const float* const* __restrict__ h_layers, int PW,
                double* __restrict__ pool_acc) {
  __shared__ int gid[GCCB_TILE_ROWS];
  const int N = node_off_v[B];
  const int tid = threadIdx.x;
  for (int tile = blockIdx.x; tile * GCCB_TILE_ROWS < N; tile += gridDim.x) {
    const int row0 = tile * GCCB_TILE_ROWS;
    __syncthreads();
    if (tid < GCCB_TILE_ROWS) gid[tid] = row0 + tid < N ? graph_id[row0 + tid] : -1;
    __syncthreads();
    for (int l = 0; l < L; ++l) {
      const int W = l == 0 ? GCCB_DINP : H;
      const float* src = l == 0 ? x0 : h_layers[l - 1];
      if (W < 128) {
        const int RGs = 256 / W > 0 ? 256 / W : 1;
        const int c = tid % W, rgs = tid / W;
        if (rgs >= RGs) continue;
        const int pers = GCCB_TILE_ROWS / RGs;
        const int rbs = rgs * pers;
        int g_run = gid[rbs];
        float acc = 0.f;
#pragma unroll 8
        for (int k = 0; k < pers; ++k) {
          const int g = gid[rbs + k];
          if (g < 0) break;
          const float x = src[(size_t)(row0 + rbs + k) * W + c];
          if (g != g_run) {
            atomicAdd(&pool_acc[((size_t)l * B + g_run) * PW + c], (double)acc);
            acc = 0.f;
            g_run = g;
          }
          acc += x;
        }
        if (g_run >= 0) atomicAdd(&pool_acc[((size_t)l * B + g_run) * PW + c], (double)acc);
        continue;
      }
      const int VW = W >> 2;
      const int RG = 256 / VW < GCCB_TILE_ROWS ? 256 / VW : GCCB_TILE_ROWS;
      const int v = tid % VW, rg = tid / VW;
      if (rg >= RG) continue;
      const int per = GCCB_TILE_ROWS / RG;
      const int rb = rg * per;
      int g_run = gid[rb];
      float4 acc = make_float4(0.f, 0.f, 0.f, 0.f);
      auto flush = [&](int g) {
        double* dst = &pool_acc[((size_t)l * B + g) * PW + 4 * v];
        atomicAdd(dst, (double)acc.x);
        atomicAdd(dst + 1, (double)acc.y);
        atomicAdd(dst + 2, (double)acc.z);
        atomicAdd(dst + 3, (double)acc.w);
      };
#pragma unroll 8
      for (int k = 0; k < per; ++k) {
        const int g = gid[rb + k];
        if (g < 0) break;
        const float4 x = *reinterpret_cast<const float4*>(src + (size_t)(row0 + rb + k) * W + 4 * v);
        if (g != g_run) {
          flush(g_run);
          acc = make_float4(0.f, 0.f, 0.f, 0.f);
          g_run = g;
        }
        acc.x += x.x; acc.y += x.y; acc.z += x.z; acc.w += x.w;
      }
      if (g_run >= 0) flush(g_run);
    }
  }
}

template <int H>
__global__ void __launch_bounds__(256)
gin_pool_predict_kernel(GinDims d, const int32_t* __restrict__ node_off_v, int B,
                        const double* __restrict__ pool_acc,
                        const float* __restrict__ params, const int64_t* __restrict__ wp_off,
                        const int64_t* __restrict__ bp_off, int PW, uint64_t drop_key,
                        uint64_t drop_step, int drop_layer_base, uint32_t keep_thresh,
                        float* __restrict__ pooled, float* __restrict__ score_out,
                        float* __restrict__ feat_out, float* __restrict__ pooled_user) {
  constexpr int MAXW = H > GCCB_DINP ? H : GCCB_DINP;
  constexpr int G = GCCB_GPB;
  __shared__ float pl[G][MAXW];
  __shared__ float score[G][H];
  const int g0 = blockIdx.x * G, tid = threadIdx.x;
  const int ng = min(G, B - g0);
  if (node_off_v[B] < 0) {
    for (int i = tid; i < ng * H; i += 256) {
      score_out[(size_t)g0 * H + i] = 0.f;
      feat_out[(size_t)g0 * H + i] = 0.f;
    }
    return;
  }
  for (int i = tid; i < G * H; i += 256) (&score[0][0])[i] = 0.f;
  __syncthreads();
  for (int l = 0; l < d.L; ++l) {
    const int W = l == 0 ? GCCB_DINP : H;
    const int inf = l == 0 ? d.din : H;
    const float* Wp = params + wp_off[l];
    const float* bp = params + bp_off[l];
    __syncthreads();
    for (int i = tid; i < G * W; i += 256) {
      const int gi = i / W, cc = i - gi * W;
      float s = 0.f;
      if (gi < ng) {
        const int g = g0 + gi;
        s = (float)pool_acc[((size_t)l * B + g) * PW + cc];
        pooled[((size_t)l * B + g) * PW + cc] = s;
        if (pooled_user && l > 0) pooled_user[((size_t)(l - 1) * B + g) * H + cc] = s;
      }
      pl[gi][cc] = s;
    }
    __syncthreads();
    for (int o0 = 0; o0 < H; o0 += 64) {
      const int o = o0 + (tid >> 2), kq = tid & 3;
      float sg[G];
#pragma unroll
      for (int gi = 0; gi < G; ++gi) sg[gi] = 0.f;
      const float* wrow = Wp + (size_t)(o < H ? o : 0) * inf;
      if (o < H) {
#pragma unroll 4
        for (int k = kq; k < inf; k += 4) {
          const float w = wrow[k];
#pragma unroll
          for (int gi = 0; gi < G; ++gi) sg[gi] = fmaf(pl[gi][k], w, sg[gi]);
        }
      }
#pragma unroll
      for (int gi = 0; gi < G; ++gi) {
        sg[gi] += __shfl_xor_sync(0xffffffffu, sg[gi], 1);
        sg[gi] += __shfl_xor_sync(0xffffffffu, sg[gi], 2);
      }
      if (kq != 0 || o >= H) continue;
      const float bias = bp[o];
#pragma unroll
      for (int gi = 0; gi < G; ++gi) {
        if (gi >= ng) break;
        float sv = sg[gi] + bias;
        if (drop_layer_base >= 0) {
          const uint32_t e = (uint32_t)((g0 + gi) * H + o);
          u32x4 w = philox_at(drop_key, drop_step, e >> 2, 0, (uint32_t)(drop_layer_base + l),
                              GCCB_TAG_DROPOUT);
          const uint32_t word = (e & 3u) == 0 ? w.x : (e & 3u) == 1 ? w.y : (e & 3u) == 2 ? w.z : w.w;
          sv = word < keep_thresh ? sv / (1.0f - d.drop_p) : 0.f;
        }
        score[gi][o] += sv;
      }
    }
    __syncthreads();
  }
  for (int gi = tid >> 5; gi < ng; gi += 8) {
    const int lane = tid & 31;
    float ss = 0.f;
    for (int o = lane; o < H; o += 32) ss = fmaf(score[gi][o], score[gi][o], ss);
    ss = warp_sum(ss);
    const float nrm = fmaxf(sqrtf(ss), d.norm_eps);
    for (int o = lane; o < H; o += 32) {
      score_out[(size_t)(g0 + gi) * H + o] = score[gi][o];
      feat_out[(size_t)(g0 + gi) * H + o] = d.norm ? score[gi][o] / nrm : score[gi][o];
    }
  }
}

template <int KIN, int H>
static size_t smem_gemm() {
  return ((size_t)GCCB_TILE_ROWS * (KIN + 1) + (size_t)GCCB_KC * (H + 4) + 2 * 16 * H + 4 * H) * sizeof(float);
}

struct FwdArgs {
  GinDims d;
  const gccb_batch_t* batch;
  int view;
  const float* pos;
  const float* params;
  gccb_gin_layout_t lay;
  float* running;
  int64_t* nbt;
  int bn_train;
  uint64_t drop_key, drop_step;
  int drop_base;
  char* acts;
  ActsLayout al;
  float* feat;
  float* pooled_user;
  const float** d_hptrs;
  int64_t* d_offs;
  gccb_stream_t stream;
};

template <int H>
static int run_forward(const FwdArgs& a) {
  const GinDims& d = a.d;
  const int B = a.batch->batch, cap = a.batch->node_cap;
  const int32_t* node_off_v = a.batch->node_off + (size_t)a.view * (B + 1);
  const int32_t* indptr = a.batch->indptr + (size_t)a.view * (cap + 1);
  const int32_t* indices = a.batch->indices + (size_t)a.view * a.batch->edge_cap;
  const int32_t* sub_deg = a.batch->sub_deg + (size_t)a.view * cap;
  const int32_t* graph_id = a.batch->graph_id + (size_t)a.view * cap;
  const float* pos_v = a.pos + (size_t)a.view * cap * d.P;
  float* x0 = (float*)(a.acts + a.al.x0);
  double* stats = (double*)(a.acts + a.al.stats);
  const int tiles = (cap + GCCB_TILE_ROWS - 1) / GCCB_TILE_ROWS;
  const int grid = tiles < 4 * GCCB_NUM_SMS ? tiles : 4 * GCCB_NUM_SMS;
  const int use_running = a.bn_train ? 0 : 1, upd = a.bn_train ? 1 : 0;
  cudaMemsetAsync(stats, 0, a.al.pool_acc + (size_t)d.L * B * a.al.PW * sizeof(double) - a.al.stats,
                  (cudaStream_t)a.stream);
  GCCB_LAUNCH(gin_build_x0_kernel, grid, 256, 0, a.stream, d, node_off_v, B, pos_v, sub_deg, graph_id,
              a.params + a.lay.emb, x0);
  const float* hin = x0;
  for (int l = 0; l < d.L - 1; ++l) {
    float* a_l = (float*)(a.acts + a.al.a[l]);
    float* z1 = (float*)(a.acts + a.al.z1[l]);
    float* z2 = (float*)(a.acts + a.al.z2[l]);
    float* hout = (float*)(a.acts + a.al.h[l]);
    double* s1 = stats + (size_t)(l * 3 + 0) * 2 * H;
    double* sa = stats + (size_t)(l * 3 + 1) * 2 * H;
    double* sb = stats + (size_t)(l * 3 + 2) * 2 * H;
    float* run1 = a.running ? a.running + (size_t)(l * 3 + 0) * 2 * H : nullptr;
    float* runa = a.running ? a.running + (size_t)(l * 3 + 1) * 2 * H : nullptr;
    float* runb = a.running ? a.running + (size_t)(l * 3 + 2) * 2 * H : nullptr;
    const float* P = a.params;
    if (l == 0) {
      auto k = gin_agg_gemm1_kernel<GCCB_DINP, H>;
      size_t sm = smem_gemm<GCCB_DINP, H>();
      gccb::ensure_dyn_smem(k, sm);
      GCCB_LAUNCH(k, grid, 256, sm, a.stream, node_off_v, B, indptr, indices, hin, P + a.lay.w1[l], d.din,
                  P + a.lay.b1[l], 0.0f, a_l, z1, s1);
    } else {
      auto k = gin_agg_gemm1_kernel<H, H>;
      size_t sm = smem_gemm<H, H>();
      gccb::ensure_dyn_smem(k, sm);
      GCCB_LAUNCH(k, grid, 256, sm, a.stream, node_off_v, B, indptr, indices, hin, P + a.lay.w1[l], H,
                  P + a.lay.b1[l], 0.0f, a_l, z1, s1);
    }
    {
      auto k = gin_bn_gemm2_kernel<H>;
      size_t sm = smem_gemm<H, H>();
      gccb::ensure_dyn_smem(k, sm);
      GCCB_LAUNCH(k, grid, 256, sm, a.stream, node_off_v, B, z1, s1, P + a.lay.bn1_w[l], P + a.lay.bn1_b[l],
                  d.bn_eps, run1, use_running, upd, d.bn_mom, P + a.lay.w2[l], P + a.lay.b2[l], z2, sa);
    }
    auto kt = gin_bn_tail_kernel<H>;
    GCCB_LAUNCH(kt, grid, 256, 0, a.stream, 0, node_off_v, B, z2, sa, P + a.lay.bna_w[l], P + a.lay.bna_b[l],
                runa, sb, P + a.lay.bnb_w[l], P + a.lay.bnb_b[l], runb, d.bn_eps, use_running, upd,
                d.bn_mom, sb, hout);
    GCCB_LAUNCH(kt, grid, 256, 0, a.stream, 1, node_off_v, B, z2, sa, P + a.lay.bna_w[l], P + a.lay.bna_b[l],
                runa, sb, P + a.lay.bnb_w[l], P + a.lay.bnb_b[l], runb, d.bn_eps, use_running, upd,
                d.bn_mom, sb, hout);
    hin = hout;
  }
  const uint32_t keep = (uint32_t)fmin((1.0 - (double)d.drop_p) * 4294967296.0, 4294967295.0);
  double* pool_acc = (double*)(a.acts + a.al.pool_acc);
  auto kpl = gin_pool_kernel<H>;
  GCCB_LAUNCH(kpl, grid, 256, 0, a.stream, d.L, node_off_v, B, graph_id, (const float*)x0, a.d_hptrs, a.al.PW,
              pool_acc);
  auto kp = gin_pool_predict_kernel<H>;
  GCCB_LAUNCH(kp, (B + GCCB_GPB - 1) / GCCB_GPB, 256, 0, a.stream, d, node_off_v, B, (const double*)pool_acc, a.params, a.d_offs, a.d_offs + 8,
              a.al.PW, a.drop_key, a.drop_step, a.drop_base, keep, (float*)(a.acts + a.al.pooled),
              (float*)(a.acts + a.al.score), a.feat, a.pooled_user);
  return check_launch("gccb_gin_forward");
}


#ifndef GCCB_EMU

__global__ void __launch_bounds__(256)
gin_cast_weights_kernel(GinDims d, gccb_gin_layout_t lay, const float* __restrict__ params, char* acts,
                        ActsLayout al) {
  const int l = blockIdx.y, H = d.H, KW = gin_kw(d, l), inf = gin_in_features(d, l);
  const float* W1 = params + lay.w1[l];
  const float* W2 = params + lay.w2[l];
  __nv_bfloat16* w1b = (__nv_bfloat16*)(acts + al.w16[l]);
  __nv_bfloat16* w2b = w1b + (size_t)H * KW;
  __nv_bfloat16* w1t = w2b + (size_t)H * H;
  __nv_bfloat16* w2t = w1t + (size_t)KW * H;
  const int n1 = H * KW, n2 = H * H;
  for (int idx = blockIdx.x * blockDim.x + threadIdx.x; idx < 2 * n1 + 2 * n2; idx += gridDim.x * blockDim.x) {
    if (idx < n1) {
      const int o = idx / KW, k = idx - o * KW;
      w1b[idx] = __float2bfloat16_rn(k < inf ? W1[(size_t)o * inf + k] : 0.f);
    } else if (idx < n1 + n2) {
      w2b[idx - n1] = __float2bfloat16_rn(W2[idx - n1]);
    } else if (idx < 2 * n1 + n2) {
      const int j = idx - n1 - n2, k = j / H, o = j - k * H;
      w1t[j] = __float2bfloat16_rn(k < inf ? W1[(size_t)o * inf + k] : 0.f);
    } else {
      const int j = idx - 2 * n1 - n2, k = j / H, o = j - k * H;
      w2t[j] = __float2bfloat16_rn(W2[(size_t)o * H + k]);
    }
  }
}

template <int W>
__global__ void __launch_bounds__(256)
gin_agg_cast_kernel(const int32_t* __restrict__ node_off_v, int B, const int32_t* __restrict__ indptr,
                    const int32_t* __restrict__ indices, const float* __restrict__ h, float eps_gin,
                    float* __restrict__ a_out, __nv_bfloat16* __restrict__ a16) {
  __shared__ float scratch[8 * W];
  __shared__ int hub_rows[GCCB_HUB_QUEUE];
  __shared__ int n_hub;
  const int N = node_off_v[B];
  const int tid = threadIdx.x, lane = tid & 31, warp = tid >> 5;
  constexpr int V4 = W / 4, PERV = (V4 + 31) / 32;
  if (tid == 0) n_hub = 0;
  __syncthreads();
  for (int r = blockIdx.x * 8 + warp; r < N; r += gridDim.x * 8) {
    const int beg = indptr[r], end = indptr[r + 1];
    if (end - beg > GCCB_HUB_DEG) {
      int slot = GCCB_HUB_QUEUE;
      if (lane == 0) slot = atomicAdd(&n_hub, 1);
      slot = __shfl_sync(0xffffffffu, slot, 0);
      if (slot < GCCB_HUB_QUEUE) {
        if (lane == 0) hub_rows[slot] = r;
        continue;
      }
    }
    float4 acc[PERV];
#pragma unroll
    for (int j = 0; j < PERV; ++j) {
      const int v = lane + 32 * j;
      acc[j] = make_float4(0.f, 0.f, 0.f, 0.f);
      if (v < V4) {
        const float4 x = *reinterpret_cast<const float4*>(h + (size_t)r * W + 4 * v);
        const float s1 = 1.0f + eps_gin;
        acc[j] = make_float4(s1 * x.x, s1 * x.y, s1 * x.z, s1 * x.w);
      }
    }
    gather_range4<W>(h, indices, beg, end, lane, acc);
#pragma unroll
    for (int j = 0; j < PERV; ++j) {
      const int v = lane + 32 * j;
      if (v < V4) {
        if (a_out) *reinterpret_cast<float4*>(a_out + (size_t)r * W + 4 * v) = acc[j];
        const __nv_bfloat162 p0 = __floats2bfloat162_rn(acc[j].x, acc[j].y), p1 = __floats2bfloat162_rn(acc[j].z, acc[j].w);
        uint2 pk;
        pk.x = *reinterpret_cast<const uint32_t*>(&p0);
        pk.y = *reinterpret_cast<const uint32_t*>(&p1);
        *reinterpret_cast<uint2*>(a16 + (size_t)r * W + 4 * v) = pk;
      }
    }
  }
  __syncthreads();
  const int nh = min(n_hub, GCCB_HUB_QUEUE);
  for (int hi = 0; hi < nh; ++hi) {
    const int rh = hub_rows[hi];
    const float sacc = gather_hub<W>(h, indices, indptr[rh], indptr[rh + 1], scratch);
    if (tid < W) {
      const float v = (1.0f + eps_gin) * h[(size_t)rh * W + tid] + sacc;
      if (a_out) a_out[(size_t)rh * W + tid] = v;
      a16[(size_t)rh * W + tid] = __float2bfloat16_rn(v);
    }
  }
}

template <int H>
__global__ void __launch_bounds__(256)
gin_bn_relu_cast_kernel(const int32_t* __restrict__ node_off_v, int B, const float* __restrict__ z1,
                        const double* __restrict__ sums1, const float* __restrict__ g1, const float* __restrict__ be1,
                        float bn_eps, float* __restrict__ running1, int use_running, int update_running,
                        float momentum, __nv_bfloat16* __restrict__ x16) {
  __shared__ float coef[4 * H];
  const int N = node_off_v[B];
  bn_prepare(sums1, N, H, g1, be1, bn_eps, coef, coef + H, coef + 2 * H, coef + 3 * H, running1, use_running != 0,
             update_running != 0, momentum);
  __syncthreads();
  const float* sc = coef + 2 * H;
  const float* sh = coef + 3 * H;
  const size_t total4 = (size_t)(N > 0 ? N : 0) * (H / 4);
  for (size_t i = (size_t)blockIdx.x * blockDim.x + threadIdx.x; i < total4; i += (size_t)gridDim.x * blockDim.x) {
    const int c = (int)(i % (H / 4)) * 4;
    const float4 z = reinterpret_cast<const float4*>(z1)[i];
    const __nv_bfloat162 p0 = __floats2bfloat162_rn(fmaxf(fmaf(z.x, sc[c], sh[c]), 0.f), fmaxf(fmaf(z.y, sc[c + 1], sh[c + 1]), 0.f));
    const __nv_bfloat162 p1 = __floats2bfloat162_rn(fmaxf(fmaf(z.z, sc[c + 2], sh[c + 2]), 0.f), fmaxf(fmaf(z.w, sc[c + 3], sh[c + 3]), 0.f));
    uint2 u;
    u.x = *reinterpret_cast<const uint32_t*>(&p0);
    u.y = *reinterpret_cast<const uint32_t*>(&p1);
    reinterpret_cast<uint2*>(x16)[i] = u;
  }
}

template <int H>
static int run_forward_tc(const FwdArgs& a) {
  const GinDims& d = a.d;
  const int B = a.batch->batch, cap = a.batch->node_cap;
  const int32_t* node_off_v = a.batch->node_off + (size_t)a.view * (B + 1);
  const int32_t* n_dev = node_off_v + B;
  const int32_t* indptr = a.batch->indptr + (size_t)a.view * (cap + 1);
  const int32_t* indices = a.batch->indices + (size_t)a.view * a.batch->edge_cap;
  const int32_t* sub_deg = a.batch->sub_deg + (size_t)a.view * cap;
  const int32_t* graph_id = a.batch->graph_id + (size_t)a.view * cap;
  const float* pos_v = a.pos + (size_t)a.view * cap * d.P;
  cudaStream_t st = (cudaStream_t)a.stream;
  float* x0 = (float*)(a.acts + a.al.x0);
  double* stats = (double*)(a.acts + a.al.stats);
  __nv_bfloat16* a16 = (__nv_bfloat16*)(a.acts + a.al.a16);
  __nv_bfloat16* x16 = (__nv_bfloat16*)(a.acts + a.al.x16);
  const int tiles = (cap + GCCB_TILE_ROWS - 1) / GCCB_TILE_ROWS;
  const int grid = tiles < 4 * GCCB_NUM_SMS ? tiles : 4 * GCCB_NUM_SMS;
  const int use_running = a.bn_train ? 0 : 1, upd = a.bn_train ? 1 : 0;
  cudaMemsetAsync(stats, 0, a.al.pool_acc + (size_t)d.L * B * a.al.PW * sizeof(double) - a.al.stats, st);
  GCCB_LAUNCH(gin_build_x0_kernel, grid, 256, 0, a.stream, d, node_off_v, B, pos_v, sub_deg, graph_id,
              a.params + a.lay.emb, x0);
  {
    dim3 gw(64, d.L - 1);
    GCCB_LAUNCH(gin_cast_weights_kernel, gw, 256, 0, a.stream, d, a.lay, a.params, a.acts, a.al);
  }
  const float* hin = x0;
  const float* P = a.params;
  const int agg_grid = tiles < 1184 ? tiles : 1184;
  for (int l = 0; l < d.L - 1; ++l) {
    float* a_l = (float*)(a.acts + a.al.a[l]);
    float* z1 = (float*)(a.acts + a.al.z1[l]);
    float* z2 = (float*)(a.acts + a.al.z2[l]);
    float* hout = (float*)(a.acts + a.al.h[l]);
    double* s1 = stats + (size_t)(l * 3 + 0) * 2 * H;
    double* sa = stats + (size_t)(l * 3 + 1) * 2 * H;
    double* sb = stats + (size_t)(l * 3 + 2) * 2 * H;
    float* run1 = a.running ? a.running + (size_t)(l * 3 + 0) * 2 * H : nullptr;
    float* runa = a.running ? a.running + (size_t)(l * 3 + 1) * 2 * H : nullptr;
    float* runb = a.running ? a.running + (size_t)(l * 3 + 2) * 2 * H : nullptr;
    const int KW = gin_kw(d, l);
    const __nv_bfloat16* w1b = (const __nv_bfloat16*)(a.acts + a.al.w16[l]);
    const __nv_bfloat16* w2b = w1b + (size_t)H * KW;
    if (l == 0) {
      auto k = gin_agg_cast_kernel<GCCB_DINP>;
      GCCB_LAUNCH(k, agg_grid, 256, 0, a.stream, node_off_v, B, indptr, indices, hin, 0.0f, a_l, a16);
    } else {
      auto k = gin_agg_cast_kernel<H>;
      GCCB_LAUNCH(k, agg_grid, 256, 0, a.stream, node_off_v, B, indptr, indices, hin, 0.0f, a_l, a16);
    }
    int rc = tc::gemm_bf16(a16, w1b, cap, H, KW, n_dev, P + a.lay.b1[l], 1.0f, z1, nullptr, H, s1, 1, nullptr, st);
    if (rc) return rc;
    auto kb = gin_bn_relu_cast_kernel<H>;
    GCCB_LAUNCH(kb, grid, 256, 0, a.stream, node_off_v, B, (const float*)z1, (const double*)s1, P + a.lay.bn1_w[l],
                P + a.lay.bn1_b[l], d.bn_eps, run1, use_running, upd, d.bn_mom, x16);
    rc = tc::gemm_bf16(x16, w2b, cap, H, H, n_dev, P + a.lay.b2[l], 1.0f, z2, nullptr, H, sa, 1, nullptr, st);
    if (rc) return rc;
    auto kt = gin_bn_tail_kernel<H>;
    GCCB_LAUNCH(kt, grid, 256, 0, a.stream, 0, node_off_v, B, z2, sa, P + a.lay.bna_w[l], P + a.lay.bna_b[l],
                runa, sb, P + a.lay.bnb_w[l], P + a.lay.bnb_b[l], runb, d.bn_eps, use_running, upd,
                d.bn_mom, sb, hout);
    GCCB_LAUNCH(kt, grid, 256, 0, a.stream, 1, node_off_v, B, z2, sa, P + a.lay.bna_w[l], P + a.lay.bna_b[l],
                runa, sb, P + a.lay.bnb_w[l], P + a.lay.bnb_b[l], runb, d.bn_eps, use_running, upd,
                d.bn_mom, sb, hout);
    hin = hout;
  }
  const uint32_t keep = (uint32_t)fmin((1.0 - (double)d.drop_p) * 4294967296.0, 4294967295.0);
  double* pool_acc = (double*)(a.acts + a.al.pool_acc);
  auto kpl = gin_pool_kernel<H>;
  GCCB_LAUNCH(kpl, grid, 256, 0, a.stream, d.L, node_off_v, B, graph_id, (const float*)x0, a.d_hptrs, a.al.PW,
              pool_acc);
  auto kp = gin_pool_predict_kernel<H>;
  GCCB_LAUNCH(kp, (B + GCCB_GPB - 1) / GCCB_GPB, 256, 0, a.stream, d, node_off_v, B, (const double*)pool_acc, a.params, a.d_offs, a.d_offs + 8,
              a.al.PW, a.drop_key, a.drop_step, a.drop_base, keep, (float*)(a.acts + a.al.pooled),
              (float*)(a.acts + a.al.score), a.feat, a.pooled_user);
  return check_launch("gccb_gin_forward (tensor cores)");
}
#endif

}

using namespace gccb;

extern "C" int gccb_gin_param_layout(const gccb_gin_cfg_t* cfg, gccb_gin_layout_t* out) {
  GinDims d;
  int rc = dims_from_cfg(cfg, &d);
  if (rc) return rc;
  if (!out) return GCCB_ERR_BADARG;
  make_param_layout(d, out);
  return GCCB_OK;
}

static size_t acts_tables_bytes() { return 256 + 8 * sizeof(void*) + 16 * sizeof(int64_t); }

extern "C" size_t gccb_gin_acts_bytes(const gccb_gin_cfg_t* cfg, int32_t batch, int32_t node_cap) {
  GinDims d;
  if (dims_from_cfg(cfg, &d)) return 0;
  return make_acts_layout(d, batch, node_cap).total + acts_tables_bytes();
}

namespace gccb {
__global__ void gin_fill_tables_kernel(char* acts, ActsLayout al, gccb_gin_layout_t lay, int L,
                                       const float** hptrs, int64_t* offs, int64_t* nbt,
                                       const int32_t* n_valid) {
  int t = threadIdx.x;
  if (t < L - 1) hptrs[t] = (const float*)(acts + al.h[t]);
  if (t < 8) { offs[t] = lay.wp[t]; offs[8 + t] = lay.bp[t]; }
  if (nbt && *n_valid >= 0 && t < 3 * (L - 1)) nbt[t] += 1;
}
}

extern "C" int gccb_gin_forward(const gccb_gin_cfg_t* cfg, const gccb_batch_t* batch, int32_t view,
                                const float* pos, const float* params, float* bn_running,
                                int64_t* num_batches_tracked, int32_t bn_train, uint64_t dropout_key,
                                uint64_t dropout_step, int32_t dropout_layer_base, void* acts,
                                size_t acts_bytes, float* feat, float* pooled_out,
                                gccb_stream_t stream) {
  FwdArgs a;
  int rc = dims_from_cfg(cfg, &a.d);
  if (rc) return rc;
  if (!batch || !pos || !params || !acts || !feat || view < 0 || view > 1 || (!bn_train && !bn_running)) {
    set_last_error("gccb_gin_forward: bad argument");
    return GCCB_ERR_BADARG;
  }
  a.al = make_acts_layout(a.d, batch->batch, batch->node_cap);
  if (acts_bytes < a.al.total + acts_tables_bytes()) {
    set_last_error("gccb_gin_forward: activation stash too small (%zu < %zu)", acts_bytes,
                   a.al.total + acts_tables_bytes());
    return GCCB_ERR_CAPACITY;
  }
  make_param_layout(a.d, &a.lay);
  a.batch = batch; a.view = view; a.pos = pos; a.params = params; a.running = bn_running;
  a.nbt = num_batches_tracked; a.bn_train = bn_train; a.drop_key = dropout_key; a.drop_step = dropout_step;
  a.drop_base = dropout_layer_base; a.acts = (char*)acts; a.feat = feat; a.pooled_user = pooled_out;
  a.stream = stream;
  char* tail = (char*)acts + a.al.total;
  a.d_hptrs = (const float**)tail;
  a.d_offs = (int64_t*)(tail + 8 * sizeof(void*));
  GCCB_LAUNCH(gin_fill_tables_kernel, 1, 32, 0, stream, (char*)acts, a.al, a.lay, a.d.L, a.d_hptrs, a.d_offs,
              bn_train ? num_batches_tracked : (int64_t*)nullptr,
              (const int32_t*)(batch->node_off + (size_t)view * (batch->batch + 1) + batch->batch));
#ifndef GCCB_EMU
  if (a.d.tc) return a.d.H == 128 ? run_forward_tc<128>(a) : run_forward_tc<256>(a);
#endif
  switch (a.d.H) {
    case 32: return run_forward<32>(a);
    case 64: return run_forward<64>(a);
    case 128: return run_forward<128>(a);
    default: return run_forward<256>(a);
  }
}
```

Baseline: 220,700.

## Fuse BN-tail reductions into the dh/aggregation kernels and move wgrad earlier on the side stream

In the backward pass, the first BN reduction pass (mode 0) is folded into the dh gather kernel through per-warp shared-memory partials and double atomics, and bn_grads launches are merged into one kernel. The W2 weight-gradient work moves to the side stream right after dz2 so it overlaps with the gemm1 backward. In the forward pass, the second bn_tail application is fused into the next layer's aggregation load and into pooling, which also write h out. The aim is fewer launches and fewer full passes over z2/dh, at the cost of more shared memory and lower occupancy in the dh kernel, plus atomic contention.

Result: no change. 226,400, median of 6 (+2.6%).

```diff
diff --git a/gcc_b200/csrc/gin_bwd.cu b/gcc_b200/csrc/gin_bwd.cu
--- a/gcc_b200/csrc/gin_bwd.cu
+++ b/gcc_b200/csrc/gin_bwd.cu
@@ -103,18 +103,52 @@
   }
 }
 
-template <int W>
-__global__ void __launch_bounds__(256)
+struct BnC { const float *mean, *invstd, *sc, *sh; };
+__device__ __forceinline__ BnC bnc(const float* p, int H) { BnC b; b.mean = p; b.invstd = p + H; b.sc = p + 2 * H; b.sh = p + 3 * H; return b; }
+
+__device__ __forceinline__ void chain_g4(float z2v, float dhv, const BnC& A, const BnC& Bc, int c,
+                                         float* ya, float* yhat, float* g4) {
+  float yap = fmaf(z2v, A.sc[c], A.sh[c]);
+  float y = fmaxf(yap, 0.f);
+  float hb = fmaf(y, Bc.sc[c], Bc.sh[c]);
+  *ya = yap;
+  *yhat = (y - Bc.mean[c]) * Bc.invstd[c];
+  *g4 = hb > 0.f ? dhv : 0.f;
+}
+
+struct RedBArgs {
+  const float* z2;
+  const double *sums_a, *sums_b;
+  const float *ga, *bea, *gb, *beb;
+  float bn_eps;
+  double* out;
+};
+
+template <int W, bool RED_B>
+__global__ void __launch_bounds__(256, !RED_B ? 8 : W > 128 ? 4 : 6)
 gin_bwd_dh_kernel(const int32_t* __restrict__ node_off_v, int B, const int32_t* __restrict__ indptr,
                   const int32_t* __restrict__ indices, const int32_t* __restrict__ graph_id,
                   const float* __restrict__ dpool_j, int DW, const float* __restrict__ da, int has_da,
-                  float* __restrict__ dh) {
+                  float* __restrict__ dh, RedBArgs rb) {
   __shared__ float scratch[8 * W];
+  __shared__ float coef[RED_B ? 8 * W : 1];
+  __shared__ float red[RED_B ? 9 * 2 * W : 1];
   __shared__ int hub_rows[GCCB_HUB_QUEUE];
   __shared__ int n_hub;
   const int N = node_off_v[B];
   const int tid = threadIdx.x, lane = tid & 31, warp = tid >> 5;
   constexpr int V4 = W / 4, PERV = (V4 + 31) / 32;
+  const float* __restrict__ z2 = rb.z2;
+  if (RED_B) {
+    bn_prepare(rb.sums_a, N, W, rb.ga, rb.bea, rb.bn_eps, coef, coef + W, coef + 2 * W, coef + 3 * W, nullptr, false,
+               false, 0.f);
+    bn_prepare(rb.sums_b, N, W, rb.gb, rb.beb, rb.bn_eps, coef + 4 * W, coef + 5 * W, coef + 6 * W, coef + 7 * W,
+               nullptr, false, false, 0.f);
+  }
+  const BnC A = bnc(coef, W), Bc = bnc(coef + 4 * W, W);
+  float* red_w = red + warp * 2 * W;
+  if (RED_B)
+    for (int i = tid; i < 8 * 2 * W; i += 256) red[i] = 0.f;
   if (tid == 0) n_hub = 0;
   __syncthreads();
   for (int r = blockIdx.x * 8 + warp; r < N; r += gridDim.x * 8) {
@@ -146,34 +180,58 @@
 #pragma unroll
     for (int j = 0; j < PERV; ++j) {
       const int v = lane + 32 * j;
-      if (v < V4) *reinterpret_cast<float4*>(dh + (size_t)r * W + 4 * v) = acc[j];
-    }
-  }
-  __syncthreads();
+      if (v < V4) {
+        *reinterpret_cast<float4*>(dh + (size_t)r * W + 4 * v) = acc[j];
+        if (RED_B) {
+          const float4 zv = *reinterpret_cast<const float4*>(z2 + (size_t)r * W + 4 * v);
+          const float zz[4] = {zv.x, zv.y, zv.z, zv.w}, dd[4] = {acc[j].x, acc[j].y, acc[j].z, acc[j].w};
+#pragma unroll
+          for (int k = 0; k < 4; ++k) {
+            const int c = 4 * v + k;
+            float ya, yhat, g4;
+            chain_g4(zz[k], dd[k], A, Bc, c, &ya, &yhat, &g4);
+            red_w[c] += g4;
+            red_w[W + c] = fmaf(g4, yhat, red_w[W + c]);
+          }
+        }
+      }
+    }
+  }
+  __syncthreads();
+  float hs = 0.f, hq = 0.f;
   const int nh = min(n_hub, GCCB_HUB_QUEUE);
   for (int hi = 0; hi < nh; ++hi) {
     const int rh = hub_rows[hi];
-    const float s = gather_hub<W>(da, indices, indptr[rh], indptr[rh + 1], scratch);
-    if (tid < W) dh[(size_t)rh * W + tid] = dpool_j[(size_t)graph_id[rh] * DW + tid] + da[(size_t)rh * W + tid] + s;
-  }
-}
-
-struct BnC { const float *mean, *invstd, *sc, *sh; };
-__device__ __forceinline__ BnC bnc(const float* p, int H) { BnC b; b.mean = p; b.invstd = p + H; b.sc = p + 2 * H; b.sh = p + 3 * H; return b; }
-
-__device__ __forceinline__ void chain_g4(float z2v, float dhv, const BnC& A, const BnC& Bc, int c,
-                                         float* ya, float* yhat, float* g4) {
-  float yap = fmaf(z2v, A.sc[c], A.sh[c]);
-  float y = fmaxf(yap, 0.f);
-  float hb = fmaf(y, Bc.sc[c], Bc.sh[c]);
-  *ya = yap;
-  *yhat = (y - Bc.mean[c]) * Bc.invstd[c];
-  *g4 = hb > 0.f ? dhv : 0.f;
+    const float sacc = gather_hub<W>(da, indices, indptr[rh], indptr[rh + 1], scratch);
+    if (tid < W) {
+      const float v = dpool_j[(size_t)graph_id[rh] * DW + tid] + da[(size_t)rh * W + tid] + sacc;
+      dh[(size_t)rh * W + tid] = v;
+      if (RED_B) {
+        float ya, yhat, g4;
+        chain_g4(z2[(size_t)rh * W + tid], v, A, Bc, tid, &ya, &yhat, &g4);
+        hs += g4;
+        hq = fmaf(g4, yhat, hq);
+      }
+    }
+  }
+  if (RED_B) {
+    if (tid < W) {
+      red[(8 * 2 + 0) * W + tid] = hs;
+      red[(8 * 2 + 1) * W + tid] = hq;
+    }
+    __syncthreads();
+    for (int idx = tid; idx < 2 * W; idx += 256) {
+      const int which = idx / W, c = idx - which * W;
+      float t = 0.f;
+      for (int w = 0; w < 9; ++w) t += red[(w * 2 + which) * W + c];
+      atomicAdd(&rb.out[which * W + c], (double)t);
+    }
+  }
 }
 
 template <int H>
 __global__ void __launch_bounds__(256)
-gin_bwd_reduce_kernel(int mode, const int32_t* __restrict__ node_off_v, int B,
+gin_bwd_reduce_kernel(const int32_t* __restrict__ node_off_v, int B,
                       const float* __restrict__ z2, const float* __restrict__ dh,
                       const double* __restrict__ sums_a, const float* __restrict__ ga,
                       const float* __restrict__ bea, const double* __restrict__ sums_b,
@@ -191,11 +249,9 @@
   constexpr int TPR = H / 4, RP = 256 / TPR;
   const int c4 = (tid % TPR) * 4, rsub = tid / TPR;
   const float invN = N > 0 ? 1.0f / (float)N : 0.f;
-  float m_g4[4] = {0.f, 0.f, 0.f, 0.f}, m_g4y[4] = {0.f, 0.f, 0.f, 0.f};
-  if (mode == 1) {
-#pragma unroll
-    for (int k = 0; k < 4; ++k) { m_g4[k] = (float)(redB_in[c4 + k] * invN); m_g4y[k] = (float)(redB_in[H + c4 + k] * invN); }
-  }
+  float m_g4[4], m_g4y[4];
+#pragma unroll
+  for (int k = 0; k < 4; ++k) { m_g4[k] = (float)(redB_in[c4 + k] * invN); m_g4y[k] = (float)(redB_in[H + c4 + k] * invN); }
   float s[4] = {0.f, 0.f, 0.f, 0.f}, q[4] = {0.f, 0.f, 0.f, 0.f};
   const int stride = gridDim.x * RP;
   for (int r = blockIdx.x * RP + rsub; r < N; r += 2 * stride) {
@@ -216,16 +272,11 @@
           const int c = c4 + k;
           float ya, yhat, g4;
           chain_g4(zz[k], dd[k], A, Bc, c, &ya, &yhat, &g4);
-          if (mode == 0) {
-            s[k] += g4;
-            q[k] = fmaf(g4, yhat, q[k]);
-          } else {
-            const float dy = Bc.sc[c] * (g4 - m_g4[k] - yhat * m_g4y[k]);
-            const float g3 = ya > 0.f ? dy : 0.f;
-            const float z2hat = (zz[k] - A.mean[c]) * A.invstd[c];
-            s[k] += g3;
-            q[k] = fmaf(g3, z2hat, q[k]);
-          }
+          const float dy = Bc.sc[c] * (g4 - m_g4[k] - yhat * m_g4y[k]);
+          const float g3 = ya > 0.f ? dy : 0.f;
+          const float z2hat = (zz[k] - A.mean[c]) * A.invstd[c];
+          s[k] += g3;
+          q[k] = fmaf(g3, z2hat, q[k]);
         }
       }
     }
@@ -510,10 +561,15 @@
   }
 }
 
-__global__ void gin_bn_grads_kernel(int H, const double* __restrict__ red, float* __restrict__ gw,
-                                    float* __restrict__ gb) {
-  int c = blockIdx.x * blockDim.x + threadIdx.x;
-  if (c < H) { gb[c] += (float)red[c]; gw[c] += (float)red[H + c]; }
+__global__ void gin_bn_grads_kernel(int H, const double* __restrict__ red, gccb_gin_layout_t lay, int l,
+                                    float* __restrict__ grads) {
+  const int i = blockIdx.x * blockDim.x + threadIdx.x;
+  if (i >= 3 * H) return;
+  const int n = i / H, c = i - n * H;
+  const int64_t w_off = n == 0 ? lay.bn1_w[l] : n == 1 ? lay.bna_w[l] : lay.bnb_w[l];
+  const int64_t b_off = n == 0 ? lay.bn1_b[l] : n == 1 ? lay.bna_b[l] : lay.bnb_b[l];
+  grads[b_off + c] += (float)red[(size_t)n * 2 * H + c];
+  grads[w_off + c] += (float)red[(size_t)n * 2 * H + H + c];
 }
 
 __global__ void __launch_bounds__(256)
@@ -585,6 +641,7 @@
   cudaEvent_t* ev_main = kit->ev;
   cudaEvent_t* ev_side = kit->ev + 8;
   cudaEvent_t ev_head = kit->ev[16], ev_join = kit->ev[17];
+  cudaEvent_t ev_gemm2 = kit->ev[18];
 #else
   gccb_stream_t side = a.stream;
 #endif
@@ -615,14 +672,13 @@
     double* r1 = red + (size_t)(l * 3 + 0) * 2 * H;
     double* rA = red + (size_t)(l * 3 + 1) * 2 * H;
     double* rB = red + (size_t)(l * 3 + 2) * 2 * H;
-    auto kdh = gin_bwd_dh_kernel<H>;
+    auto kdh = gin_bwd_dh_kernel<H, true>;
     GCCB_LAUNCH(kdh, (tiles < 1184 ? tiles : 1184), 256, 0, a.stream, node_off_v, B, indptr, indices, graph_id,
-                (const float*)(dpool + (size_t)j * B * DW), DW, (const float*)da, j < d.L - 1 ? 1 : 0, dh);
+                (const float*)(dpool + (size_t)j * B * DW), DW, (const float*)da, j < d.L - 1 ? 1 : 0, dh,
+                RedBArgs{z2, sa, sb, P + a.lay.bna_w[l], P + a.lay.bna_b[l], P + a.lay.bnb_w[l], P + a.lay.bnb_b[l],
+                         d.bn_eps, rB});
     auto kred = gin_bwd_reduce_kernel<H>;
-    GCCB_LAUNCH(kred, grid, 256, 0, a.stream, 0, node_off_v, B, z2, (const float*)dh, sa, P + a.lay.bna_w[l],
-                P + a.lay.bna_b[l], sb, P + a.lay.bnb_w[l], P + a.lay.bnb_b[l], d.bn_eps,
-                (const double*)rB, rB);
-    GCCB_LAUNCH(kred, grid, 256, 0, a.stream, 1, node_off_v, B, z2, (const float*)dh, sa, P + a.lay.bna_w[l],
+    GCCB_LAUNCH(kred, grid, 256, 0, a.stream, node_off_v, B, z2, (const float*)dh, sa, P + a.lay.bna_w[l],
                 P + a.lay.bna_b[l], sb, P + a.lay.bnb_w[l], P + a.lay.bnb_b[l], d.bn_eps,
                 (const double*)rB, rA);
 #ifndef GCCB_EMU
@@ -637,6 +693,18 @@
                   P + a.lay.bnb_b[l], d.bn_eps, (const double*)rB, (const double*)rA, P + a.lay.w2[l], dz2,
                   g1, r1);
     }
+#ifndef GCCB_EMU
+    cudaEventRecord(ev_gemm2, main_s);
+    cudaStreamWaitEvent((cudaStream_t)side, ev_gemm2, 0);
+#endif
+    {
+      dim3 gr(GCCB_WG_CHUNKS, ((H + 63) / 64) * ((H + 63) / 64));
+      GCCB_LAUNCH(gin_wgrad_kernel, gr, 256, 0, side, node_off_v, B, H, H, (const float*)dz2, z1, s1,
+                  P + a.lay.bn1_w[l], P + a.lay.bn1_b[l], d.bn_eps, part);
+      GCCB_LAUNCH(gin_wgrad_reduce_kernel, (H * H + H + 255) / 256, 256, 0, side, H, H, H,
+                  (const float*)part, G + a.lay.w2[l], G + a.lay.b2[l]);
+    }
+    GCCB_LAUNCH(gin_bn_grads_kernel, (3 * H + 127) / 128, 128, 0, side, H, (const double*)r1, a.lay, l, G);
     const int KQ1 = gin_in_width(d, l), inf = gin_in_features(d, l);
     if (l == 0) {
       auto k = gin_bwd_gemm1_kernel<GCCB_DINP, H>;
@@ -656,30 +724,19 @@
     cudaStreamWaitEvent((cudaStream_t)side, ev_main[l], 0);
 #endif
     {
-      dim3 gr(GCCB_WG_CHUNKS, ((H + 63) / 64) * ((H + 63) / 64));
-      GCCB_LAUNCH(gin_wgrad_kernel, gr, 256, 0, side, node_off_v, B, H, H, (const float*)dz2, z1, s1,
-                  P + a.lay.bn1_w[l], P + a.lay.bn1_b[l], d.bn_eps, part);
-      GCCB_LAUNCH(gin_wgrad_reduce_kernel, (H * H + H + 255) / 256, 256, 0, side, H, H, H,
-                  (const float*)part, G + a.lay.w2[l], G + a.lay.b2[l]);
       dim3 gr1(GCCB_WG_CHUNKS, ((H + 63) / 64) * ((KQ1 + 63) / 64));
       GCCB_LAUNCH(gin_wgrad_kernel, gr1, 256, 0, side, node_off_v, B, H, KQ1, (const float*)g1, a_l,
                   (const double*)nullptr, (const float*)nullptr, (const float*)nullptr, d.bn_eps, part);
       GCCB_LAUNCH(gin_wgrad_reduce_kernel, (H * KQ1 + H + 255) / 256, 256, 0, side, H, KQ1, inf,
                   (const float*)part, G + a.lay.w1[l], G + a.lay.b1[l]);
     }
-    GCCB_LAUNCH(gin_bn_grads_kernel, (H + 127) / 128, 128, 0, side, H, (const double*)rB,
-                G + a.lay.bnb_w[l], G + a.lay.bnb_b[l]);
-    GCCB_LAUNCH(gin_bn_grads_kernel, (H + 127) / 128, 128, 0, side, H, (const double*)rA,
-                G + a.lay.bna_w[l], G + a.lay.bna_b[l]);
-    GCCB_LAUNCH(gin_bn_grads_kernel, (H + 127) / 128, 128, 0, side, H, (const double*)r1,
-                G + a.lay.bn1_w[l], G + a.lay.bn1_b[l]);
 #ifndef GCCB_EMU
     cudaEventRecord(ev_side[l], (cudaStream_t)side);
 #endif
   }
-  auto kdh0 = gin_bwd_dh_kernel<GCCB_DINP>;
+  auto kdh0 = gin_bwd_dh_kernel<GCCB_DINP, false>;
   GCCB_LAUNCH(kdh0, (tiles < 1184 ? tiles : 1184), 256, 0, a.stream, node_off_v, B, indptr, indices, graph_id, (const float*)dpool, DW,
-              (const float*)da, 1, dh);
+              (const float*)da, 1, dh, RedBArgs{});
   {
     size_t sm = (size_t)(d.maxdeg + 1) * d.D * sizeof(float);
     auto k = gin_bwd_emb_kernel;
@@ -935,13 +992,13 @@
     const __nv_bfloat16* w1t = w1b + (size_t)H * KW + (size_t)H * H;
     const __nv_bfloat16* w2t = w1t + (size_t)KW * H;
     float* c1 = coef1 + (size_t)l * 2 * H;
-    auto kdh = gin_bwd_dh_kernel<H>;
+    auto kdh = gin_bwd_dh_kernel<H, true>;
     GCCB_LAUNCH(kdh, (tiles < 1184 ? tiles : 1184), 256, 0, a.stream, node_off_v, B, indptr, indices, graph_id,
-                (const float*)(dpool + (size_t)j * B * DW), DW, (const float*)da, j < d.L - 1 ? 1 : 0, dh);
+                (const float*)(dpool + (size_t)j * B * DW), DW, (const float*)da, j < d.L - 1 ? 1 : 0, dh,
+                RedBArgs{z2, sa, sb, P + a.lay.bna_w[l], P + a.lay.bna_b[l], P + a.lay.bnb_w[l], P + a.lay.bnb_b[l],
+                         d.bn_eps, rB});
     auto kred = gin_bwd_reduce_kernel<H>;
-    GCCB_LAUNCH(kred, grid, 256, 0, a.stream, 0, node_off_v, B, z2, (const float*)dh, sa, P + a.lay.bna_w[l],
-                P + a.lay.bna_b[l], sb, P + a.lay.bnb_w[l], P + a.lay.bnb_b[l], d.bn_eps, (const double*)rB, rB);
-    GCCB_LAUNCH(kred, grid, 256, 0, a.stream, 1, node_off_v, B, z2, (const float*)dh, sa, P + a.lay.bna_w[l],
+    GCCB_LAUNCH(kred, grid, 256, 0, a.stream, node_off_v, B, z2, (const float*)dh, sa, P + a.lay.bna_w[l],
                 P + a.lay.bna_b[l], sb, P + a.lay.bnb_w[l], P + a.lay.bnb_b[l], d.bn_eps, (const double*)rB, rA);
     if (l + 2 <= d.L - 2) cudaStreamWaitEvent(main_s, ev_side[l + 2], 0);
     auto kz2 = gin_bwd_dz2_kernel<H>;
@@ -969,17 +1026,12 @@
     if (!rc) rc = tc::gemm_bf16(tA, tB, H, KW, capP, nullptr, nullptr, 1.0f, G + a.lay.w1[l], nullptr, inf, nullptr,
                                 a.bl.splits, splitk, side, 1.0f, inf);
     if (rc) return rc;
-    GCCB_LAUNCH(gin_bn_grads_kernel, (H + 127) / 128, 128, 0, side, H, (const double*)rB,
-                G + a.lay.bnb_w[l], G + a.lay.bnb_b[l]);
-    GCCB_LAUNCH(gin_bn_grads_kernel, (H + 127) / 128, 128, 0, side, H, (const double*)rA,
-                G + a.lay.bna_w[l], G + a.lay.bna_b[l]);
-    GCCB_LAUNCH(gin_bn_grads_kernel, (H + 127) / 128, 128, 0, side, H, (const double*)r1,
-                G + a.lay.bn1_w[l], G + a.lay.bn1_b[l]);
+    GCCB_LAUNCH(gin_bn_grads_kernel, (3 * H + 127) / 128, 128, 0, side, H, (const double*)r1, a.lay, l, G);
     cudaEventRecord(ev_side[l], side);
   }
-  auto kdh0 = gin_bwd_dh_kernel<GCCB_DINP>;
+  auto kdh0 = gin_bwd_dh_kernel<GCCB_DINP, false>;
   GCCB_LAUNCH(kdh0, (tiles < 1184 ? tiles : 1184), 256, 0, a.stream, node_off_v, B, indptr, indices, graph_id, (const float*)dpool, DW,
-              (const float*)da, 1, dh);
+              (const float*)da, 1, dh, RedBArgs{});
   {
     size_t sm = (size_t)(d.maxdeg + 1) * d.D * sizeof(float);
     auto k = gin_bwd_emb_kernel;
diff --git a/gcc_b200/csrc/gin_common.cuh b/gcc_b200/csrc/gin_common.cuh
--- a/gcc_b200/csrc/gin_common.cuh
+++ b/gcc_b200/csrc/gin_common.cuh
@@ -1,4 +1,6 @@
 #pragma once
+#include <type_traits>
+
 #include "common.cuh"
 
 namespace gccb {
@@ -185,14 +187,51 @@
   }
 }
 
+struct GinBnTail {
+  const float* z2;
+  const double *sums_a, *sums_b;
+  const float *ga, *bea, *gb, *beb;
+  float *running_a, *running_b;
+  float eps, momentum;
+  int use_running, update_running_b;
+};
+
+__device__ __forceinline__ void bn_tail_prepare(const GinBnTail& t, int N, int H, float* coef) {
+  bn_prepare(t.sums_a, N, H, t.ga, t.bea, t.eps, coef, coef + H, coef + 2 * H, coef + 3 * H, t.running_a,
+             t.use_running != 0, false, t.momentum);
+  bn_prepare(t.sums_b, N, H, t.gb, t.beb, t.eps, coef + 4 * H, coef + 5 * H, coef + 6 * H, coef + 7 * H,
+             t.running_b, t.use_running != 0, t.update_running_b != 0, t.momentum);
+}
+
+struct LoadAsIs {
+  __device__ __forceinline__ LoadAsIs() {}
+  __device__ __forceinline__ LoadAsIs(const float*, int) {}
+  __device__ __forceinline__ float operator()(float x, int) const { return x; }
+};
+struct LoadBnTail {
+  const float *sca, *sha, *scb, *shb;
+  __device__ __forceinline__ LoadBnTail(const float* coef, int H)
+      : sca(coef + 2 * H), sha(coef + 3 * H), scb(coef + 6 * H), shb(coef + 7 * H) {}
+  __device__ __forceinline__ float operator()(float z, int c) const {
+    const float y = fmaxf(fmaf(z, sca[c], sha[c]), 0.f);
+    return fmaxf(fmaf(y, scb[c], shb[c]), 0.f);
+  }
+};
+template <class XF>
+__device__ __forceinline__ float4 load_xf4(const float* p, int c, XF xf) {
+  const float4 x = *reinterpret_cast<const float4*>(p);
+  return make_float4(xf(x.x, c), xf(x.y, c + 1), xf(x.z, c + 2), xf(x.w, c + 3));
+}
+
 #ifndef GCCB_HUB_DEG
 #define GCCB_HUB_DEG 256
 #endif
 #define GCCB_GPB 8
 #define GCCB_HUB_QUEUE 64
-template <int W>
+template <int W, class XF = LoadAsIs>
 __device__ __forceinline__ void gather_range(const float* __restrict__ src, const int32_t* __restrict__ indices,
-                                             int beg, int end, int lane, float (&acc)[(W + 31) / 32]) {
+                                             int beg, int end, int lane, float (&acc)[(W + 31) / 32],
+                                             XF xf = XF()) {
   constexpr int PER = (W + 31) / 32;
   int e = beg;
   for (; e + 7 < end; e += 8) {
@@ -205,7 +244,7 @@
       if (c < W) {
         float x[8];
 #pragma unroll
-        for (int k = 0; k < 8; ++k) x[k] = src[(size_t)u[k] * W + c];
+        for (int k = 0; k < 8; ++k) x[k] = xf(src[(size_t)u[k] * W + c], c);
         acc[j] += ((x[0] + x[1]) + (x[2] + x[3])) + ((x[4] + x[5]) + (x[6] + x[7]));
       }
     }
@@ -215,14 +254,15 @@
 #pragma unroll
     for (int j = 0; j < PER; ++j) {
       const int c = lane + 32 * j;
-      if (c < W) acc[j] += src[(size_t)u * W + c];
+      if (c < W) acc[j] += xf(src[(size_t)u * W + c], c);
     }
   }
 }
 
-template <int W>
+template <int W, class XF = LoadAsIs>
 __device__ __forceinline__ void gather_range4(const float* __restrict__ src, const int32_t* __restrict__ indices,
-                                              int beg, int end, int lane, float4 (&acc)[(W / 4 + 31) / 32]) {
+                                              int beg, int end, int lane, float4 (&acc)[(W / 4 + 31) / 32],
+                                              XF xf = XF()) {
   constexpr int V4 = W / 4, PERV = (V4 + 31) / 32;
   int e = beg;
   for (; e + 3 < end; e += 4) {
@@ -231,10 +271,10 @@
     for (int j = 0; j < PERV; ++j) {
       const int v = lane + 32 * j;
       if (v < V4) {
-        const float4 x0 = *reinterpret_cast<const float4*>(src + (size_t)u0 * W + 4 * v);
-        const float4 x1 = *reinterpret_cast<const float4*>(src + (size_t)u1 * W + 4 * v);
-        const float4 x2 = *reinterpret_cast<const float4*>(src + (size_t)u2 * W + 4 * v);
-        const float4 x3 = *reinterpret_cast<const float4*>(src + (size_t)u3 * W + 4 * v);
+        const float4 x0 = load_xf4(src + (size_t)u0 * W + 4 * v, 4 * v, xf);
+        const float4 x1 = load_xf4(src + (size_t)u1 * W + 4 * v, 4 * v, xf);
+        const float4 x2 = load_xf4(src + (size_t)u2 * W + 4 * v, 4 * v, xf);
+        const float4 x3 = load_xf4(src + (size_t)u3 * W + 4 * v, 4 * v, xf);
         acc[j].x += (x0.x + x1.x) + (x2.x + x3.x);
         acc[j].y += (x0.y + x1.y) + (x2.y + x3.y);
         acc[j].z += (x0.z + x1.z) + (x2.z + x3.z);
@@ -248,16 +288,16 @@
     for (int j = 0; j < PERV; ++j) {
       const int v = lane + 32 * j;
       if (v < V4) {
-        const float4 x = *reinterpret_cast<const float4*>(src + (size_t)u * W + 4 * v);
+        const float4 x = load_xf4(src + (size_t)u * W + 4 * v, 4 * v, xf);
         acc[j].x += x.x; acc[j].y += x.y; acc[j].z += x.z; acc[j].w += x.w;
       }
     }
   }
 }
 
-template <int W>
+template <int W, class XF = LoadAsIs>
 __device__ __forceinline__ float gather_hub(const float* __restrict__ src, const int32_t* __restrict__ indices,
-                                            int beg, int end, float* scratch) {
+                                            int beg, int end, float* scratch, XF xf = XF()) {
   constexpr int PER = (W + 31) / 32;
   const int lane = threadIdx.x & 31, warp = threadIdx.x >> 5;
   const int len = end - beg, per = (len + 7) / 8;
@@ -265,7 +305,7 @@
   float acc[PER];
 #pragma unroll
   for (int j = 0; j < PER; ++j) acc[j] = 0.f;
-  gather_range<W>(src, indices, b, e > b ? e : b, lane, acc);
+  gather_range<W>(src, indices, b, e > b ? e : b, lane, acc, xf);
 #pragma unroll
   for (int j = 0; j < PER; ++j) {
     const int c = lane + 32 * j;
diff --git a/gcc_b200/csrc/gin_fwd.cu b/gcc_b200/csrc/gin_fwd.cu
--- a/gcc_b200/csrc/gin_fwd.cu
+++ b/gcc_b200/csrc/gin_fwd.cu
@@ -29,25 +29,31 @@
   }
 }
 
-template <int KIN, int H>
+template <int KIN, int H, bool BN_IN>
 __global__ void __launch_bounds__(256)
 gin_agg_gemm1_kernel(const int32_t* __restrict__ node_off_v, int B, const int32_t* __restrict__ indptr,
-                     const int32_t* __restrict__ indices, const float* __restrict__ h,
-                     const float* __restrict__ W1, int in_features, const float* __restrict__ b1,
-                     float eps_gin, float* __restrict__ a_out, float* __restrict__ z1,
+                     const int32_t* __restrict__ indices, const float* __restrict__ x0, GinBnTail prev,
+                     float* __restrict__ h_out, const float* __restrict__ W1, int in_features,
+                     const float* __restrict__ b1, float eps_gin, float* __restrict__ a_out, float* __restrict__ z1,
                      double* __restrict__ sums) {
   GCCB_DYN_SMEM(float, smem);
   constexpr int LDA = KIN + 1;
   float* As = smem;
   float* Ws = As + GCCB_TILE_ROWS * LDA;
   float* red = Ws + GCCB_KC * (H + 4);
+  float* coef = red + 2 * 16 * H;
   __shared__ int hub_rows[GCCB_TILE_ROWS];
   __shared__ int n_hub;
   static_assert(8 * KIN <= 2 * 16 * H, "hub scratch must fit in the statistics scratch");
+  static_assert(!BN_IN || KIN == H, "a previous layer's output is H wide");
   const int N = node_off_v[B];
   const int tid = threadIdx.x, lane = tid & 31, warp = tid >> 5;
   const int tx = tid & 15, ty = tid >> 4;
   using TC = TileCols<H>;
+  using XF = typename std::conditional<BN_IN, LoadBnTail, LoadAsIs>::type;
+  const float* h = BN_IN ? prev.z2 : x0;
+  if (BN_IN) bn_tail_prepare(prev, N, KIN, coef);
+  const XF xf(coef, KIN);
   for (int tile = blockIdx.x; tile * GCCB_TILE_ROWS < N; tile += gridDim.x) {
     const int row0 = tile * GCCB_TILE_ROWS;
     __syncthreads();
@@ -68,9 +74,13 @@
 #pragma unroll
         for (int j = 0; j < PER; ++j) {
           int c = lane + 32 * j;
-          if (c < KIN) acc[j] = (1.0f + eps_gin) * h[(size_t)r * KIN + c];
-        }
-        gather_range<KIN>(h, indices, beg, end, lane, acc);
+          if (c < KIN) {
+            const float hv = xf(h[(size_t)r * KIN + c], c);
+            if (BN_IN) h_out[(size_t)r * KIN + c] = hv;
+            acc[j] = (1.0f + eps_gin) * hv;
+          }
+        }
+        gather_range<KIN>(h, indices, beg, end, lane, acc, xf);
       }
 #pragma unroll
       for (int j = 0; j < PER; ++j) {
@@ -84,9 +94,11 @@
     __syncthreads();
     for (int hi = 0; hi < n_hub; ++hi) {
       const int rr = hub_rows[hi], r = row0 + rr;
-      const float s = gather_hub<KIN>(h, indices, indptr[r], indptr[r + 1], red);
+      const float s = gather_hub<KIN>(h, indices, indptr[r], indptr[r + 1], red, xf);
       if (tid < KIN) {
-        const float v = (1.0f + eps_gin) * h[(size_t)r * KIN + tid] + s;
+        const float hv = xf(h[(size_t)r * KIN + tid], tid);
+        if (BN_IN) h_out[(size_t)r * KIN + tid] = hv;
+        const float v = (1.0f + eps_gin) * hv + s;
         As[rr * LDA + tid] = v;
         a_out[(size_t)r * KIN + tid] = v;
       }
@@ -165,23 +177,17 @@
 
 template <int H>
 __global__ void __launch_bounds__(256)
-gin_bn_tail_kernel(int mode, const int32_t* __restrict__ node_off_v, int B,
+gin_bn_tail_kernel(const int32_t* __restrict__ node_off_v, int B,
                    const float* __restrict__ z2, const double* __restrict__ sums_a,
                    const float* __restrict__ ga, const float* __restrict__ bea,
-                   float* __restrict__ running_a, const double* __restrict__ sums_b_in,
-                   const float* __restrict__ gb, const float* __restrict__ beb,
-                   float* __restrict__ running_b, float bn_eps, int use_running, int update_running,
-                   float momentum, double* __restrict__ sums_b_out, float* __restrict__ h_out) {
+                   float* __restrict__ running_a, float bn_eps, int use_running, int update_running,
+                   float momentum, double* __restrict__ sums_b_out) {
   __shared__ float coef_a[4 * H];
-  __shared__ float coef_b[4 * H];
   __shared__ float red[2 * 1024];
   const int N = node_off_v[B];
   const int tid = threadIdx.x;
   bn_prepare(sums_a, N, H, ga, bea, bn_eps, coef_a, coef_a + H, coef_a + 2 * H, coef_a + 3 * H,
-             running_a, use_running != 0, update_running != 0 && mode == 0, momentum);
-  if (mode == 1)
-    bn_prepare(sums_b_in, N, H, gb, beb, bn_eps, coef_b, coef_b + H, coef_b + 2 * H, coef_b + 3 * H,
-               running_b, use_running != 0, update_running != 0, momentum);
+             running_a, use_running != 0, update_running != 0, momentum);
   __syncthreads();
   constexpr int TPR = H / 4, RP = 256 / TPR;
   const int c4 = (tid % TPR) * 4, rsub = tid / TPR;
@@ -189,77 +195,52 @@
 #pragma unroll
   for (int k = 0; k < 4; ++k) { sca[k] = coef_a[2 * H + c4 + k]; sha[k] = coef_a[3 * H + c4 + k]; }
   const int stride = gridDim.x * RP;
-  if (mode == 0) {
-    float s[4] = {0.f, 0.f, 0.f, 0.f}, q[4] = {0.f, 0.f, 0.f, 0.f};
-    for (int r = blockIdx.x * RP + rsub; r < N; r += 4 * stride) {
-      float4 z[4];
-#pragma unroll
-      for (int u = 0; u < 4; ++u) {
-        const int rr = r + u * stride;
-        z[u] = rr < N ? *reinterpret_cast<const float4*>(z2 + (size_t)rr * H + c4) : make_float4(0.f, 0.f, 0.f, 0.f);
-      }
-#pragma unroll
-      for (int u = 0; u < 4; ++u) {
-        if (r + u * stride < N) {
-          const float zz[4] = {z[u].x, z[u].y, z[u].z, z[u].w};
-#pragma unroll
-          for (int k = 0; k < 4; ++k) {
-            const float y = fmaxf(fmaf(zz[k], sca[k], sha[k]), 0.f);
-            s[k] += y;
-            q[k] = fmaf(y, y, q[k]);
-          }
-        }
-      }
-    }
-#pragma unroll
-    for (int k = 0; k < 4; ++k) {
-      red[(0 * RP + rsub) * H + c4 + k] = s[k];
-      red[(RP + rsub) * H + c4 + k] = q[k];
-    }
-    __syncthreads();
-    for (int idx = tid; idx < 2 * H; idx += 256) {
-      int which = idx / H, cc = idx - which * H;
-      float t = 0.f;
-      for (int j = 0; j < RP; ++j) t += red[(which * RP + j) * H + cc];
-      atomicAdd(&sums_b_out[which * H + cc], (double)t);
-    }
-  } else {
-    float scb[4], shb[4];
-#pragma unroll
-    for (int k = 0; k < 4; ++k) { scb[k] = coef_b[2 * H + c4 + k]; shb[k] = coef_b[3 * H + c4 + k]; }
-    for (int r = blockIdx.x * RP + rsub; r < N; r += 4 * stride) {
-      float4 z[4];
-#pragma unroll
-      for (int u = 0; u < 4; ++u) {
-        const int rr = r + u * stride;
-        z[u] = rr < N ? *reinterpret_cast<const float4*>(z2 + (size_t)rr * H + c4) : make_float4(0.f, 0.f, 0.f, 0.f);
-      }
-#pragma unroll
-      for (int u = 0; u < 4; ++u) {
-        const int rr = r + u * stride;
-        if (rr < N) {
-          const float zz[4] = {z[u].x, z[u].y, z[u].z, z[u].w};
-          float o[4];
-#pragma unroll
-          for (int k = 0; k < 4; ++k) {
-            const float y = fmaxf(fmaf(zz[k], sca[k], sha[k]), 0.f);
-            o[k] = fmaxf(fmaf(y, scb[k], shb[k]), 0.f);
-          }
-          *reinterpret_cast<float4*>(h_out + (size_t)rr * H + c4) = make_float4(o[0], o[1], o[2], o[3]);
-        }
-      }
-    }
+  float s[4] = {0.f, 0.f, 0.f, 0.f}, q[4] = {0.f, 0.f, 0.f, 0.f};
+  for (int r = blockIdx.x * RP + rsub; r < N; r += 4 * stride) {
+    float4 z[4];
+#pragma unroll
+    for (int u = 0; u < 4; ++u) {
+      const int rr = r + u * stride;
+      z[u] = rr < N ? *reinterpret_cast<const float4*>(z2 + (size_t)rr * H + c4) : make_float4(0.f, 0.f, 0.f, 0.f);
+    }
+#pragma unroll
+    for (int u = 0; u < 4; ++u) {
+      if (r + u * stride < N) {
+        const float zz[4] = {z[u].x, z[u].y, z[u].z, z[u].w};
+#pragma unroll
+        for (int k = 0; k < 4; ++k) {
+          const float y = fmaxf(fmaf(zz[k], sca[k], sha[k]), 0.f);
+          s[k] += y;
+          q[k] = fmaf(y, y, q[k]);
+        }
+      }
+    }
+  }
+#pragma unroll
+  for (int k = 0; k < 4; ++k) {
+    red[(0 * RP + rsub) * H + c4 + k] = s[k];
+    red[(RP + rsub) * H + c4 + k] = q[k];
+  }
+  __syncthreads();
+  for (int idx = tid; idx < 2 * H; idx += 256) {
+    int which = idx / H, cc = idx - which * H;
+    float t = 0.f;
+    for (int j = 0; j < RP; ++j) t += red[(which * RP + j) * H + cc];
+    atomicAdd(&sums_b_out[which * H + cc], (double)t);
   }
 }
 
 template <int H>
 __global__ void __launch_bounds__(256)
 gin_pool_kernel(int L, const int32_t* __restrict__ node_off_v, int B, const int32_t* __restrict__ graph_id,
-                const float* __restrict__ x0, const float* const* __restrict__ h_layers, int PW,
-                double* __restrict__ pool_acc) {
+                const float* __restrict__ x0, const float* const* __restrict__ h_layers, GinBnTail last,
+                float* __restrict__ h_last, int PW, double* __restrict__ pool_acc) {
   __shared__ int gid[GCCB_TILE_ROWS];
+  __shared__ float coef[8 * H];
   const int N = node_off_v[B];
   const int tid = threadIdx.x;
+  bn_tail_prepare(last, N, H, coef);
+  const LoadBnTail xf(coef, H);
   for (int tile = blockIdx.x; tile * GCCB_TILE_ROWS < N; tile += gridDim.x) {
     const int row0 = tile * GCCB_TILE_ROWS;
     __syncthreads();
@@ -267,7 +248,8 @@
     __syncthreads();
     for (int l = 0; l < L; ++l) {
       const int W = l == 0 ? GCCB_DINP : H;
-      const float* src = l == 0 ? x0 : h_layers[l - 1];
+      const bool from_z2 = l == L - 1;
+      const float* src = l == 0 ? x0 : from_z2 ? last.z2 : h_layers[l - 1];
       if (W < 128) {
         const int RGs = 256 / W > 0 ? 256 / W : 1;
         const int c = tid % W, rgs = tid / W;
@@ -280,7 +262,12 @@
         for (int k = 0; k < pers; ++k) {
           const int g = gid[rbs + k];
           if (g < 0) break;
-          const float x = src[(size_t)(row0 + rbs + k) * W + c];
+          const size_t at = (size_t)(row0 + rbs + k) * W + c;
+          float x = src[at];
+          if (from_z2) {
+            x = xf(x, c);
+            h_last[at] = x;
+          }
           if (g != g_run) {
             atomicAdd(&pool_acc[((size_t)l * B + g_run) * PW + c], (double)acc);
             acc = 0.f;
@@ -310,7 +297,12 @@
       for (int k = 0; k < per; ++k) {
         const int g = gid[rb + k];
         if (g < 0) break;
-        const float4 x = *reinterpret_cast<const float4*>(src + (size_t)(row0 + rb + k) * W + 4 * v);
+        const size_t at = (size_t)(row0 + rb + k) * W + 4 * v;
+        float4 x = *reinterpret_cast<const float4*>(src + at);
+        if (from_z2) {
+          x = make_float4(xf(x.x, 4 * v), xf(x.y, 4 * v + 1), xf(x.z, 4 * v + 2), xf(x.w, 4 * v + 3));
+          *reinterpret_cast<float4*>(h_last + at) = x;
+        }
         if (g != g_run) {
           flush(g_run);
           acc = make_float4(0.f, 0.f, 0.f, 0.f);
@@ -416,8 +408,9 @@
 }
 
 template <int KIN, int H>
-static size_t smem_gemm() {
-  return ((size_t)GCCB_TILE_ROWS * (KIN + 1) + (size_t)GCCB_KC * (H + 4) + 2 * 16 * H + 4 * H) * sizeof(float);
+static size_t smem_gemm(int bn_bundles) {
+  return ((size_t)GCCB_TILE_ROWS * (KIN + 1) + (size_t)GCCB_KC * (H + 4) + 2 * 16 * H + (size_t)bn_bundles * 4 * KIN) *
+         sizeof(float);
 }
 
 struct FwdArgs {
@@ -441,6 +434,26 @@
   gccb_stream_t stream;
 };
 
+static GinBnTail bn_tail_args(const FwdArgs& a, int l) {
+  const int H = a.d.H;
+  const double* stats = (const double*)(a.acts + a.al.stats);
+  GinBnTail t;
+  t.z2 = (const float*)(a.acts + a.al.z2[l]);
+  t.sums_a = stats + (size_t)(l * 3 + 1) * 2 * H;
+  t.sums_b = stats + (size_t)(l * 3 + 2) * 2 * H;
+  t.ga = a.params + a.lay.bna_w[l];
+  t.bea = a.params + a.lay.bna_b[l];
+  t.gb = a.params + a.lay.bnb_w[l];
+  t.beb = a.params + a.lay.bnb_b[l];
+  t.running_a = a.running ? a.running + (size_t)(l * 3 + 1) * 2 * H : nullptr;
+  t.running_b = a.running ? a.running + (size_t)(l * 3 + 2) * 2 * H : nullptr;
+  t.eps = a.d.bn_eps;
+  t.momentum = a.d.bn_mom;
+  t.use_running = a.bn_train ? 0 : 1;
+  t.update_running_b = a.bn_train ? 1 : 0;
+  return t;
+}
+
 template <int H>
 static int run_forward(const FwdArgs& a) {
   const GinDims& d = a.d;
@@ -460,53 +473,46 @@
                   (cudaStream_t)a.stream);
   GCCB_LAUNCH(gin_build_x0_kernel, grid, 256, 0, a.stream, d, node_off_v, B, pos_v, sub_deg, graph_id,
               a.params + a.lay.emb, x0);
-  const float* hin = x0;
   for (int l = 0; l < d.L - 1; ++l) {
     float* a_l = (float*)(a.acts + a.al.a[l]);
     float* z1 = (float*)(a.acts + a.al.z1[l]);
     float* z2 = (float*)(a.acts + a.al.z2[l]);
-    float* hout = (float*)(a.acts + a.al.h[l]);
     double* s1 = stats + (size_t)(l * 3 + 0) * 2 * H;
     double* sa = stats + (size_t)(l * 3 + 1) * 2 * H;
     double* sb = stats + (size_t)(l * 3 + 2) * 2 * H;
     float* run1 = a.running ? a.running + (size_t)(l * 3 + 0) * 2 * H : nullptr;
     float* runa = a.running ? a.running + (size_t)(l * 3 + 1) * 2 * H : nullptr;
-    float* runb = a.running ? a.running + (size_t)(l * 3 + 2) * 2 * H : nullptr;
     const float* P = a.params;
     if (l == 0) {
-      auto k = gin_agg_gemm1_kernel<GCCB_DINP, H>;
-      size_t sm = smem_gemm<GCCB_DINP, H>();
+      auto k = gin_agg_gemm1_kernel<GCCB_DINP, H, false>;
+      size_t sm = smem_gemm<GCCB_DINP, H>(0);
       gccb::ensure_dyn_smem(k, sm);
-      GCCB_LAUNCH(k, grid, 256, sm, a.stream, node_off_v, B, indptr, indices, hin, P + a.lay.w1[l], d.din,
-                  P + a.lay.b1[l], 0.0f, a_l, z1, s1);
+      GCCB_LAUNCH(k, grid, 256, sm, a.stream, node_off_v, B, indptr, indices, (const float*)x0, GinBnTail{},
+                  (float*)nullptr, P + a.lay.w1[l], d.din, P + a.lay.b1[l], 0.0f, a_l, z1, s1);
     } else {
-      auto k = gin_agg_gemm1_kernel<H, H>;
-      size_t sm = smem_gemm<H, H>();
+      auto k = gin_agg_gemm1_kernel<H, H, true>;
+      size_t sm = smem_gemm<H, H>(2);
       gccb::ensure_dyn_smem(k, sm);
-      GCCB_LAUNCH(k, grid, 256, sm, a.stream, node_off_v, B, indptr, indices, hin, P + a.lay.w1[l], H,
-                  P + a.lay.b1[l], 0.0f, a_l, z1, s1);
+      GCCB_LAUNCH(k, grid, 256, sm, a.stream, node_off_v, B, indptr, indices, (const float*)nullptr,
+                  bn_tail_args(a, l - 1), (float*)(a.acts + a.al.h[l - 1]), P + a.lay.w1[l], H, P + a.lay.b1[l],
+                  0.0f, a_l, z1, s1);
     }
     {
       auto k = gin_bn_gemm2_kernel<H>;
-      size_t sm = smem_gemm<H, H>();
+      size_t sm = smem_gemm<H, H>(1);
       gccb::ensure_dyn_smem(k, sm);
       GCCB_LAUNCH(k, grid, 256, sm, a.stream, node_off_v, B, z1, s1, P + a.lay.bn1_w[l], P + a.lay.bn1_b[l],
                   d.bn_eps, run1, use_running, upd, d.bn_mom, P + a.lay.w2[l], P + a.lay.b2[l], z2, sa);
     }
     auto kt = gin_bn_tail_kernel<H>;
-    GCCB_LAUNCH(kt, grid, 256, 0, a.stream, 0, node_off_v, B, z2, sa, P + a.lay.bna_w[l], P + a.lay.bna_b[l],
-                runa, sb, P + a.lay.bnb_w[l], P + a.lay.bnb_b[l], runb, d.bn_eps, use_running, upd,
-                d.bn_mom, sb, hout);
-    GCCB_LAUNCH(kt, grid, 256, 0, a.stream, 1, node_off_v, B, z2, sa, P + a.lay.bna_w[l], P + a.lay.bna_b[l],
-                runa, sb, P + a.lay.bnb_w[l], P + a.lay.bnb_b[l], runb, d.bn_eps, use_running, upd,
-                d.bn_mom, sb, hout);
-    hin = hout;
+    GCCB_LAUNCH(kt, grid, 256, 0, a.stream, node_off_v, B, z2, sa, P + a.lay.bna_w[l], P + a.lay.bna_b[l],
+                runa, d.bn_eps, use_running, upd, d.bn_mom, sb);
   }
   const uint32_t keep = (uint32_t)fmin((1.0 - (double)d.drop_p) * 4294967296.0, 4294967295.0);
   double* pool_acc = (double*)(a.acts + a.al.pool_acc);
   auto kpl = gin_pool_kernel<H>;
-  GCCB_LAUNCH(kpl, grid, 256, 0, a.stream, d.L, node_off_v, B, graph_id, (const float*)x0, a.d_hptrs, a.al.PW,
-              pool_acc);
+  GCCB_LAUNCH(kpl, grid, 256, 0, a.stream, d.L, node_off_v, B, graph_id, (const float*)x0, a.d_hptrs,
+              bn_tail_args(a, d.L - 2), (float*)(a.acts + a.al.h[d.L - 2]), a.al.PW, pool_acc);
   auto kp = gin_pool_predict_kernel<H>;
   GCCB_LAUNCH(kp, (B + GCCB_GPB - 1) / GCCB_GPB, 256, 0, a.stream, d, node_off_v, B, (const double*)pool_acc, a.params, a.d_offs, a.d_offs + 8,
               a.al.PW, a.drop_key, a.drop_step, a.drop_base, keep, (float*)(a.acts + a.al.pooled),
@@ -544,17 +550,23 @@
   }
 }
 
-template <int W>
+template <int W, bool BN_IN>
 __global__ void __launch_bounds__(256)
 gin_agg_cast_kernel(const int32_t* __restrict__ node_off_v, int B, const int32_t* __restrict__ indptr,
-                    const int32_t* __restrict__ indices, const float* __restrict__ h, float eps_gin,
-                    float* __restrict__ a_out, __nv_bfloat16* __restrict__ a16) {
+                    const int32_t* __restrict__ indices, const float* __restrict__ x0, GinBnTail prev,
+                    float* __restrict__ h_out, float eps_gin, float* __restrict__ a_out,
+                    __nv_bfloat16* __restrict__ a16) {
   __shared__ float scratch[8 * W];
+  __shared__ float coef[BN_IN ? 8 * W : 1];
   __shared__ int hub_rows[GCCB_HUB_QUEUE];
   __shared__ int n_hub;
   const int N = node_off_v[B];
   const int tid = threadIdx.x, lane = tid & 31, warp = tid >> 5;
   constexpr int V4 = W / 4, PERV = (V4 + 31) / 32;
+  using XF = typename std::conditional<BN_IN, LoadBnTail, LoadAsIs>::type;
+  const float* h = BN_IN ? prev.z2 : x0;
+  if (BN_IN) bn_tail_prepare(prev, N, W, coef);
+  const XF xf(coef, W);
   if (tid == 0) n_hub = 0;
   __syncthreads();
   for (int r = blockIdx.x * 8 + warp; r < N; r += gridDim.x * 8) {
@@ -574,12 +586,13 @@
       const int v = lane + 32 * j;
       acc[j] = make_float4(0.f, 0.f, 0.f, 0.f);
       if (v < V4) {
-        const float4 x = *reinterpret_cast<const float4*>(h + (size_t)r * W + 4 * v);
+        const float4 x = load_xf4(h + (size_t)r * W + 4 * v, 4 * v, xf);
+        if (BN_IN) *reinterpret_cast<float4*>(h_out + (size_t)r * W + 4 * v) = x;
         const float s1 = 1.0f + eps_gin;
         acc[j] = make_float4(s1 * x.x, s1 * x.y, s1 * x.z, s1 * x.w);
       }
     }
-    gather_range4<W>(h, indices, beg, end, lane, acc);
+    gather_range4<W>(h, indices, beg, end, lane, acc, xf);
 #pragma unroll
     for (int j = 0; j < PERV; ++j) {
       const int v = lane + 32 * j;
@@ -597,9 +610,11 @@
   const int nh = min(n_hub, GCCB_HUB_QUEUE);
   for (int hi = 0; hi < nh; ++hi) {
     const int rh = hub_rows[hi];
-    const float sacc = gather_hub<W>(h, indices, indptr[rh], indptr[rh + 1], scratch);
+    const float sacc = gather_hub<W>(h, indices, indptr[rh], indptr[rh + 1], scratch, xf);
     if (tid < W) {
-      const float v = (1.0f + eps_gin) * h[(size_t)rh * W + tid] + sacc;
+      const float hv = xf(h[(size_t)rh * W + tid], tid);
+      if (BN_IN) h_out[(size_t)rh * W + tid] = hv;
+      const float v = (1.0f + eps_gin) * hv + sacc;
       if (a_out) a_out[(size_t)rh * W + tid] = v;
       a16[(size_t)rh * W + tid] = __float2bfloat16_rn(v);
     }
@@ -658,29 +673,28 @@
     dim3 gw(64, d.L - 1);
     GCCB_LAUNCH(gin_cast_weights_kernel, gw, 256, 0, a.stream, d, a.lay, a.params, a.acts, a.al);
   }
-  const float* hin = x0;
   const float* P = a.params;
   const int agg_grid = tiles < 1184 ? tiles : 1184;
   for (int l = 0; l < d.L - 1; ++l) {
     float* a_l = (float*)(a.acts + a.al.a[l]);
     float* z1 = (float*)(a.acts + a.al.z1[l]);
     float* z2 = (float*)(a.acts + a.al.z2[l]);
-    float* hout = (float*)(a.acts + a.al.h[l]);
     double* s1 = stats + (size_t)(l * 3 + 0) * 2 * H;
     double* sa = stats + (size_t)(l * 3 + 1) * 2 * H;
     double* sb = stats + (size_t)(l * 3 + 2) * 2 * H;
     float* run1 = a.running ? a.running + (size_t)(l * 3 + 0) * 2 * H : nullptr;
     float* runa = a.running ? a.running + (size_t)(l * 3 + 1) * 2 * H : nullptr;
-    float* runb = a.running ? a.running + (size_t)(l * 3 + 2) * 2 * H : nullptr;
     const int KW = gin_kw(d, l);
     const __nv_bfloat16* w1b = (const __nv_bfloat16*)(a.acts + a.al.w16[l]);
     const __nv_bfloat16* w2b = w1b + (size_t)H * KW;
     if (l == 0) {
-      auto k = gin_agg_cast_kernel<GCCB_DINP>;
-      GCCB_LAUNCH(k, agg_grid, 256, 0, a.stream, node_off_v, B, indptr, indices, hin, 0.0f, a_l, a16);
+      auto k = gin_agg_cast_kernel<GCCB_DINP, false>;
+      GCCB_LAUNCH(k, agg_grid, 256, 0, a.stream, node_off_v, B, indptr, indices, (const float*)x0, GinBnTail{},
+                  (float*)nullptr, 0.0f, a_l, a16);
     } else {
-      auto k = gin_agg_cast_kernel<H>;
-      GCCB_LAUNCH(k, agg_grid, 256, 0, a.stream, node_off_v, B, indptr, indices, hin, 0.0f, a_l, a16);
+      auto k = gin_agg_cast_kernel<H, true>;
+      GCCB_LAUNCH(k, agg_grid, 256, 0, a.stream, node_off_v, B, indptr, indices, (const float*)nullptr,
+                  bn_tail_args(a, l - 1), (float*)(a.acts + a.al.h[l - 1]), 0.0f, a_l, a16);
     }
     int rc = tc::gemm_bf16(a16, w1b, cap, H, KW, n_dev, P + a.lay.b1[l], 1.0f, z1, nullptr, H, s1, 1, nullptr, st);
     if (rc) return rc;
@@ -690,19 +704,14 @@
     rc = tc::gemm_bf16(x16, w2b, cap, H, H, n_dev, P + a.lay.b2[l], 1.0f, z2, nullptr, H, sa, 1, nullptr, st);
     if (rc) return rc;
     auto kt = gin_bn_tail_kernel<H>;
-    GCCB_LAUNCH(kt, grid, 256, 0, a.stream, 0, node_off_v, B, z2, sa, P + a.lay.bna_w[l], P + a.lay.bna_b[l],
-                runa, sb, P + a.lay.bnb_w[l], P + a.lay.bnb_b[l], runb, d.bn_eps, use_running, upd,
-                d.bn_mom, sb, hout);
-    GCCB_LAUNCH(kt, grid, 256, 0, a.stream, 1, node_off_v, B, z2, sa, P + a.lay.bna_w[l], P + a.lay.bna_b[l],
-                runa, sb, P + a.lay.bnb_w[l], P + a.lay.bnb_b[l], runb, d.bn_eps, use_running, upd,
-                d.bn_mom, sb, hout);
-    hin = hout;
+    GCCB_LAUNCH(kt, grid, 256, 0, a.stream, node_off_v, B, z2, sa, P + a.lay.bna_w[l], P + a.lay.bna_b[l],
+                runa, d.bn_eps, use_running, upd, d.bn_mom, sb);
   }
   const uint32_t keep = (uint32_t)fmin((1.0 - (double)d.drop_p) * 4294967296.0, 4294967295.0);
   double* pool_acc = (double*)(a.acts + a.al.pool_acc);
   auto kpl = gin_pool_kernel<H>;
-  GCCB_LAUNCH(kpl, grid, 256, 0, a.stream, d.L, node_off_v, B, graph_id, (const float*)x0, a.d_hptrs, a.al.PW,
-              pool_acc);
+  GCCB_LAUNCH(kpl, grid, 256, 0, a.stream, d.L, node_off_v, B, graph_id, (const float*)x0, a.d_hptrs,
+              bn_tail_args(a, d.L - 2), (float*)(a.acts + a.al.h[d.L - 2]), a.al.PW, pool_acc);
   auto kp = gin_pool_predict_kernel<H>;
   GCCB_LAUNCH(kp, (B + GCCB_GPB - 1) / GCCB_GPB, 256, 0, a.stream, d, node_off_v, B, (const double*)pool_acc, a.params, a.d_offs, a.d_offs + 8,
               a.al.PW, a.drop_key, a.drop_step, a.drop_base, keep, (float*)(a.acts + a.al.pooled),
```
